# ZeningLin/ViBERTgrid-PyTorch

Hardware: AMD Instinct MI355X
Metric: training docs/sec, 512x512 img + seq_len 512, bert-base+resnet34; 1/2/4/8 GPU (higher is better)
Workload: dtype f32

## Files before the change

### include/vbg.h

```cpp
#ifndef VBG_H
#define VBG_H

#ifdef __cplusplus
extern "C" {
#endif

#define VBG_VERSION 100

int vbg_version(void);

enum {
    VBG_OP_DENSE_K = 0,
    VBG_OP_DENSE_R = 1,
    VBG_OP_CONV_K = 2,
    VBG_OP_CONV_R = 3,
    VBG_OP_WT_R = 4
};
enum { VBG_EPI_NONE = 0, VBG_EPI_RELU = 1, VBG_EPI_GELU_DUAL = 2 ,
       VBG_EPI_MUL_GELU_GRAD = 3  };

typedef struct vbg_conv_geo {
    int Hs, Ws, Cs;
    int Hr, Wr;
    int kh, kw, stride, pad;
// ... 40 lines not shown
    const unsigned short* A; long long a_plane; long long lda;
    const unsigned short* B; long long b_plane; long long ldb;
    float* C; long long ldc; float* C2; const float* bias;
    unsigned short* Cp; long long c_plane; long long ldp;
    int epi; float alpha; int accumulate;
    int splitk;
    int tile;
    int trans;
    int ngroups;
    vbg_plane_group grp[VBG_PLANE_MAX_GROUPS];
    float* colsum;
    int form;
    unsigned short* Cq; long long q_plane; long long ldq;
    const unsigned* a_amax;
    unsigned* c_amax;
    const unsigned* cq_ref_in; const unsigned* cq_l1_in; float cq_mul; unsigned* cq_ref_out;
} vbg_plane_gemm_desc;
typedef struct vbg_l1_entry { const float* w; long long ld; int rows, cols; } vbg_l1_entry;
int vbg_col_l1_max(const vbg_l1_entry* table_dev, int n, int max_cols, unsigned* out, void* stream);
int vbg_plane_gemm(const vbg_plane_gemm_desc* desc, void* stream);
int vbg_plane_gemm_timed(const vbg_plane_gemm_desc* desc, void* stream, void* start_event, void* stop_event);
int vbg_split_planes(const float* x, long long ldx, int rows, int cols, unsigned short* out, int ldp, long long plane, int relu,
                     float* colsum_accum, void* stream);
int vbg_split_planes_t(const float* x, long long ldx, int rows, int cols, unsigned short* out, int ldp, long long plane,
                       void* stream);
int vbg_split_planes_pair(const float* x, long long ldx, int rows, int cols, unsigned short* out, int ldp, long long plane,
                          const unsigned* amax, float* colsum_accum, void* stream);
int vbg_split_planes_t_batched(const float* src, unsigned short* dst, const long long* tbl_dev, int njobs, int total_tiles,
                               long long plane, void* stream);
int vbg_split_planes_pair_t_batched(const float* src, unsigned short* dst, const long long* tbl_dev, int njobs, int total_tiles,
                                    long long plane, void* stream);

enum { VBG_ATTN_FWD = 0, VBG_ATTN_DQ = 1, VBG_ATTN_DKV = 2 };
typedef struct vbg_attn_desc {
    int mode, heads, ntasks, max_len;
    const int* tasks; const int* seq_len; const int* seq_row0; const int* pad_off; long long ntok_pad;
    const unsigned short* qkv; long long qkv_plane, qkv_ld;
    const unsigned short* dO; long long do_plane, do_ld;
    float* out; long long ldo;
    float* lse; float* delta;
    unsigned short* out_planes; long long op_plane, op_ld;
    float* kbar; long long ldk;
    const float* o;
    const unsigned* mask_q; const unsigned* mask_k; const long long* mask_off;
    float scale, keep_scale;
    unsigned* out_amax;
    unsigned short* out_pair; long long oq_plane, oq_ld;
    int form;
    const unsigned* do_amax;
} vbg_attn_desc;
int vbg_attn(const vbg_attn_desc* desc, void* stream);
unsigned vbg_attn_drop_thr16(float drop_p);
int vbg_attn_mask(const int* seq_len, const long long* mask_off, int nseq, int heads, int maxlen, float drop_p,
                  unsigned long long seed, unsigned long long stream_id, unsigned* mask_q, unsigned* mask_k, void* stream);
int vbg_attn_mask_layers(const int* seq_len, const long long* mask_off, int nseq, int heads, int maxlen, float drop_p,
                         unsigned long long seed, unsigned long long stream_id0, unsigned long long stream_id_stride, int nlayers,
                         long long layer_words, unsigned* mask_q, unsigned* mask_k, void* stream);

int vbg_colsum(const float* x, long long ld, int M, int N, float* out, int accumulate, void* stream);
int vbg_colsum_f64(const float* x, long long ld, int M, int N, float* out, int accumulate, double* ws, void* stream);

int vbg_conv3x3_split(int B, int H, int W, int Cs, int N);
int vbg_conv3x3(const float* x, const float* w, const float* bias, float* y, double* stats, int stats_slots, int B, int H, int W,
                int Cs, int N, int accumulate, int form, const unsigned* x_amax, float* split_slab, unsigned* split_tickets,
                int nsplit, void* stream);
#define VBG_AMAX_WORDS 64
#define VBG_AMAX_STRIDE 32
int vbg_amax(const float* x, long long n, unsigned* amax, void* stream);
int vbg_conv3x3_wflip(const float* w, int Cout, int Cin, float* out, void* stream);

typedef struct vbg_conv3_wprep_entry {
    const float* w;
    void* out;
    int Cout, Cin, flip, bn;
} vbg_conv3_wprep_entry;
long long vbg_conv3x3_wprep_bytes(int Cout, int Cin, int flip, int bn);
int vbg_conv3x3_wprep(const vbg_conv3_wprep_entry* table_dev, const vbg_conv3_wprep_entry* table_host, int n, void* stream);
int vbg_conv3x3_pw(const float* x, const void* w_planes, const float* bias, float* y, double* stats, int stats_slots, int B, int H, int W,
                   int Cs, int N, int accumulate, const unsigned* x_amax, float* split_slab, unsigned* split_tickets, int nsplit,
                   int bn, void* stream);
int vbg_conv3x3_pw_amp(const float* x, const void* w_planes, const float* bias, float* y, double* stats, int stats_slots, int B, int H, int W,
                       int Cs, int N, int accumulate, const unsigned* x_amax, float* split_slab, unsigned* split_tickets, int nsplit,
                       int bn, void* stream);

int vbg_conv3x3_wgrad_strips(int B, int H, int W, int Cs, int Cout);
int vbg_conv3x3_wgrad(const float* dy, const float* x, float* dw, float* slab, int B, int H, int W, int Cs, int Cout, int form,
                      const unsigned* dy_amax, const unsigned* x_amax, void* stream);

int vbg_im2col(const float* x, int B, int H, int W, int C, int kh, int kw, int stride, int pad, int Kpad,
               float* out, void* stream);

int vbg_normalize_resize(const float* img, int h, int w, int oh, int ow, const float* h_mean3, const float* h_std3,
                         float* batch_nhwc, int b, int H, int W, void* stream);
int vbg_rescale_boxes(const long long* in, int S, float ratio_h, float ratio_w, int* out, void* stream);

int vbg_embed_ln_fwd(const int* ids, const int* pos_ids, int ntok, int hidden, const float* word, const float* pos,
                     const float* type0, const float* gamma, const float* beta, float eps, float drop_p,
                     unsigned long long seed, unsigned long long stream_id, float* out, float* xhat, float* rstd,
                     void* stream);
int vbg_embed_ln_bwd(const float* dout, const float* xhat, const float* rstd, const int* ids, const int* pos_ids,
                     int ntok, int hidden, const float* gamma, float drop_p, unsigned long long seed,
                     unsigned long long stream_id, float* dword, float* dpos, float* dtype0, float* dgamma,
                     float* dbeta, void* stream);
int vbg_dropout_add_ln_fwd(const float* x, const float* res, int rows, int hidden, const float* gamma,
                           const float* beta, float eps, float drop_p, unsigned long long seed,
                           unsigned long long stream_id, float* y, float* xhat, float* rstd, void* stream);
int vbg_dropout_add_ln_fwd_planes(const float* x, const float* res, int rows, int hidden, const float* gamma,
                                  const float* beta, float eps, float drop_p, unsigned long long seed,
                                  unsigned long long stream_id, float* y, float* xhat, float* rstd, unsigned short* y_planes, int ldp,
                                  long long plane, unsigned short* y_pair, int ldq, long long qplane, void* stream);
int vbg_ln_bwd_ws_rows(int rows);
int vbg_dropout_add_ln_bwd(const float* dy, const float* xhat, const float* rstd, int rows, int hidden,
                           const float* gamma, float drop_p, unsigned long long seed, unsigned long long stream_id,
                           float* dx, float* dres, float* dgamma, float* dbeta, float* slots_ws, unsigned* dx_amax, void* stream);
int vbg_dropout_add_ln_bwd_planes(const float* dy, const float* xhat, const float* rstd, int rows, int hidden,
                                  const float* gamma, float drop_p, unsigned long long seed, unsigned long long stream_id,
                                  unsigned short* dx_planes, int ldp, long long plane, float* dres, float* dgamma, float* dbeta,
                                  float* dbias_accum, float* slots3_ws, void* stream);
int vbg_dropout_add_ln_bwd_pair(const float* dy, const float* xhat, const float* rstd, int rows, int hidden,
                                const float* gamma, float drop_p, unsigned long long seed, unsigned long long stream_id,
                                unsigned short* dx_pair, int ldp, long long plane, float* dres, float* dgamma, float* dbeta,
                                float* dbias_accum, float* slots3_ws, const unsigned* dy_amax, unsigned* dx_amax, unsigned* dx_bound,
                                void* stream);
int vbg_softmax_fwd(float* s, const long long* off, const int* len, const int* ldp, int ngroups, int heads,
                    int maxlen, float scale, float drop_p, unsigned long long seed, unsigned long long stream_id,
                    void* stream);
int vbg_softmax_bwd(const float* p, float* dp, const long long* off, const int* len, const int* ldp, int ngroups,
                    int heads, int maxlen, float scale, float drop_p, void* stream);
int vbg_row_softmax(const float* x, int rows, int cols, float* y, void* stream);
int vbg_gelu_bwd(const float* h, float* dg_inout, long long n, void* stream);
int vbg_relu_bwd(const float* y, float* dy_inout, long long n, void* stream);

typedef struct vbg_planes_ref { unsigned short* buf; long long plane, ld; } vbg_planes_ref;
typedef struct vbg_bert_layer_fwd_desc {
    int ntok, hidden, inter, heads;
    float eps, drop_p; unsigned long long seed, stream_id0;
    int form_qkv, form_attn, form_ao, form_ffn;
    int tile_qkv, tile_ao, tile_ffn1, tile_ffn2;
    int ntasks, max_len; const int* tasks; const int* seq_len; const int* seq_row0; const int* pad_off; long long ntok_pad;
    const unsigned* mask_q; const unsigned* mask_k; const long long* mask_off; float attn_scale, keep_scale;
    const float* x; vbg_planes_ref xa;
    vbg_planes_ref wqkv, wo, wi, wo2;
    const float* bqkv; const float* bo; const float* bi; const float* bo2; const float* g1; const float* b1; const float* g2; const float* b2;
    vbg_planes_ref pqkv;
    float* ctx; float* lse; float* kbar; vbg_planes_ref pctx, pctxq;
    float* ao; float* x1; float* xhat1; float* rstd1; vbg_planes_ref px1, px1q;
    float* h; vbg_planes_ref pg, pgq;
    float* fo; float* y; float* xhat2; float* rstd2; vbg_planes_ref py, pyq;
} vbg_bert_layer_fwd_desc;
int vbg_bert_layer_fwd(const vbg_bert_layer_fwd_desc* desc, void* stream);

int vbg_seg_reduce_fwd(const float* tok, const int* tok_row, const int* run_start, const int* run_len, int nseg,
                       int hidden, int mode, float* out, void* stream);
int vbg_seg_reduce_bwd(const float* dout, const int* tok_row, const int* run_start, const int* run_len, int nseg,
                       int hidden, int mode, float* dtok_accum, void* stream);

int vbg_owner_map(const int* boxes, const int* box_off, int B, int gh, int gw, int stride, int* owner, void* stream);
int vbg_grid_scatter_fwd(const float* emb, const int* owner, int B, int gh, int gw, int C, int layout, float* grid,
                         void* stream);
int vbg_grid_scatter_bwd(const float* dgrid, const int* owner, const int* boxes, const int* box_doc, int nbox, int gh,
                         int gw, int stride, int C, float* demb_accum, void* stream);
int vbg_label_raster(const int* owner, const int* seg_class, long long ncell, int* pos_neg, int* cls, void* stream);

int vbg_bn_slots(void);
int vbg_bn_stats(const float* x, long long M, int C, double* slots_accum, void* stream);
int vbg_bn_finalize(double* stats, int nslots, int clear_slots, double count, const double* count_dev, int C, float eps, float momentum,
                    float* mean, float* invstd, float* running_mean, float* running_var, void* stream);
int vbg_bn_apply(const float* x, const float* res, long long M, int C, const float* mean, const float* invstd,
                 const float* gamma, const float* beta, int relu, float* y, unsigned* y_amax, void* stream);
int vbg_bn_bwd_reduce(const float* dy, const float* y, const float* x, long long M, int C, const float* mean,
                      const float* invstd, int relu, double* slots_accum, void* stream);
int vbg_bn_bwd_apply(const float* dy, const float* y, const float* x, long long M, int C, const float* mean,
                     const float* invstd, const float* gamma, const double* sums, double count, const double* count_dev,
                     int relu, float* dx,
                     float* dres, float* dgamma_accum, float* dbeta_accum, unsigned* dx_amax, void* stream);
int vbg_bn_apply_fold(const float* x, const float* res, long long M, int C, double* slots, int nslots, double count,
                      const double* count_dev, float eps, float momentum, float* mean, float* invstd, float* running_mean,
                      float* running_var, const float* gamma, const float* beta, int relu, float* y, unsigned* y_amax, void* stream);
int vbg_bn_fold_count(double* slots, int nslots, int clear_slots, int C, double* folded, double count, void* stream);
int vbg_bn_bwd_apply_fold(const float* dy, const float* y, const float* x, long long M, int C, const float* mean,
                          const float* invstd, const float* gamma, double* slots, int nslots, double count, int relu, float* dx,
                          float* dres, float* dgamma_accum, float* dbeta_accum, unsigned* dx_amax, void* stream);
int vbg_bn_param_grad(double* slots, int nslots, int clear_slots, int C, double* folded, float* dgamma_accum, float* dbeta_accum,
                      void* stream);
int vbg_maxpool3x3s2_fwd(const float* x, int B, int H, int W, int C, float* y, int* argmax, void* stream);
int vbg_maxpool3x3s2_bwd(const float* dy, const int* argmax, int B, int Ho, int Wo, int C, int H, int W,
                         float* dx, void* stream);
int vbg_avgpool2_fwd(const float* x, int B, int H, int W, int C, float* y, void* stream);
int vbg_avgpool2_bwd(const float* dy, int B, int H, int W, int C, float* dx, void* stream);
int vbg_upsample2_add(const float* lo, const float* skip, int B, int H, int W, int C, float* y, void* stream);
int vbg_sumpool(const float* hi, int B, int H, int W, int C, int f, float* lo, int accumulate, void* stream);
int vbg_nchw_to_nhwc(const float* x, int B, int C, int HW, float* y, void* stream);
int vbg_nhwc_to_nchw(const float* x, int B, int C, int HW, float* y, void* stream);
int vbg_upsample_nhwc_to_nchw(const float* x, int B, int h, int w, int C, int f, float* y, void* stream);
int vbg_add_inplace(float* a, const float* b, long long n, void* stream);

int vbg_roi_align_fwd(const float* feat, int B, int H, int W, int C, const int* boxes, const int* box_doc, int nroi,
                      int out, float scale, float* y , void* stream);
int vbg_roi_align_bwd(const float* dy, int B, int H, int W, int C, const int* boxes, const int* box_doc, int nroi,
                      int out, float scale, float* dfeat_accum, void* stream);

int vbg_ce_fwd(const float* logits, long long ld, int ncls, const int* elem, const int* labels, long long n,
               const float* weight, int up_shift, int H, int W, float* loss, void* stream);
int vbg_ce_bwd(const float* logits, long long ld, int ncls, const int* elem, const int* labels, long long n,
               const float* weight, const float* gscale_dev, float gmul, int up_shift, int H, int W,
               float* dlogits_accum, void* stream);
long long vbg_compact_ws_bytes(long long n);
int vbg_compact(const int* labels, long long n, int value, int eq, int* out_idx, int* out_count_dev, void* ws,
                long long ws_bytes, void* stream);
long long vbg_sort_ws_bytes(long long n);
int vbg_sort_desc(const float* keys, long long n, float* keys_out, int* idx_out, void* ws, long long ws_bytes,
                  void* stream);
int vbg_gather_f32(const float* src, const int* idx, long long n, float* out, void* stream);
int vbg_gather_i32(const int* src, const int* idx, long long n, int* out, void* stream);
int vbg_sum_f32(const float* x, long long n, float* out_accum, void* stream);

int vbg_gather_rows(const float* src, const int* idx, long long n, int C, float* dst, void* stream);
int vbg_scatter_rows_add(const float* src, const int* idx, long long n, int C, float* dst_accum, void* stream);
int vbg_crf_nll_fwd(const float* emissions, const int* tags, const int* doc_off, int ndoc, const float* trans, int ntag,
                    int start_tag, int stop_tag, float* alpha, float* logz, float* nll, void* stream);
int vbg_crf_nll_bwd(const float* emissions, const int* tags, const int* doc_off, int ndoc, const float* trans, int ntag,
                    int start_tag, int stop_tag, const float* alpha, const float* logz, const float* gout, float* demissions,
                    float* dtrans_accum, void* stream);
int vbg_crf_viterbi(const float* emissions, const int* doc_off, int ndoc, const float* trans, int ntag, int start_tag,
                    int stop_tag, int* backptr, int* path, float* score, void* stream);

int vbg_sgd_step(float* p, const float* g, float* mom, long long n, float lr, float momentum, float wd,
                 int first_step, float grad_scale, void* stream);
int vbg_adamw_step(float* p, const float* g, float* m, float* v, long long n, float lr, float b1, float b2,
                   float eps, float wd, int step, float grad_scale, void* stream);
int vbg_sumsq(const float* g, long long n, float* out_accum, void* stream);
int vbg_scale_inplace(float* x, long long n, float s, void* stream);

#ifdef __cplusplus
}
#endif
#endif
```

### vibertgrid-pytorch_amd/csrc/conv3.hip

```cpp
#include "vbg_common.h"
#include <type_traits>
#include <stdlib.h>
#include "../../include/vbg.h"

namespace vbg {

typedef unsigned c3_u32x4 __attribute__((ext_vector_type(4)));
typedef __bf16 c3_bf16x8 __attribute__((ext_vector_type(8)));
constexpr unsigned C3_INVALID = 0x80000000u;

struct conv3_args {
    const float* X;
    const float* Wt;
    const unsigned short* Wp;
    const float* bias;
    float* Y;
    double* stats;
    int stats_slots;
    int H, W, wsh, Cs, N, M;
    int roi;
    int ksplit, csplit;
    float* slab;
    unsigned* tickets;
    int accumulate;
    const unsigned* a_amax;
};

__device__ __forceinline__ __amdgpu_buffer_rsrc_t c3_rsrc(const float* base) {
    return __builtin_amdgcn_make_buffer_rsrc(const_cast<float*>(base), 0, (int)0x80000000u, 0x00020000);
}
__device__ __forceinline__ float4 c3_load(__amdgpu_buffer_rsrc_t r, unsigned vo) {
    const c3_u32x4 v = __builtin_amdgcn_raw_buffer_load_b128(r, (int)vo, 0, 0);
    return make_float4(__uint_as_float(v[0]), __uint_as_float(v[1]), __uint_as_float(v[2]), __uint_as_float(v[3]));
}
__device__ __forceinline__ void c3_split3(float a, float b, unsigned& hi, unsigned& mid, unsigned& lo) {
    const float ra = a - __uint_as_float(__float_as_uint(a) & 0xffff0000u), rb = b - __uint_as_float(__float_as_uint(b) & 0xffff0000u);
    const float sa = ra - __uint_as_float(__float_as_uint(ra) & 0xffff0000u), sb = rb - __uint_as_float(__float_as_uint(rb) & 0xffff0000u);
    hi = __builtin_amdgcn_perm(__float_as_uint(b), __float_as_uint(a), 0x07060302u);
    mid = __builtin_amdgcn_perm(__float_as_uint(rb), __float_as_uint(ra), 0x07060302u);
    lo = __builtin_amdgcn_perm(__float_as_uint(sb), __float_as_uint(sa), 0x07060302u);
}
typedef _Float16 c3_f16x8 __attribute__((ext_vector_type(8)));
typedef __fp16 c3_f16x2 __attribute__((ext_vector_type(2)));
__device__ __forceinline__ void c3_split2(float a, float b, unsigned& hi, unsigned& lo) {
    typedef float f32x2_t __attribute__((ext_vector_type(2)));
    typedef _Float16 f16x2_t __attribute__((ext_vector_type(2)));
    const f32x2_t v = {a, b};
    const f16x2_t h = __builtin_convertvector(v, f16x2_t);
    const f16x2_t l = __builtin_convertvector((v - __builtin_convertvector(h, f32x2_t)) * 2048.f, f16x2_t);
    hi = __builtin_bit_cast(unsigned, h);
    lo = __builtin_bit_cast(unsigned, l);
}
__device__ __forceinline__ unsigned c3_amax_read(const unsigned* slot) {
    unsigned v = slot[(threadIdx.x & (VBG_AMAX_WORDS - 1)) * VBG_AMAX_STRIDE];
#pragma unroll
    for (int o = 32; o > 0; o >>= 1) v = max(v, (unsigned)__shfl_xor((int)v, o, 64));
    return __builtin_amdgcn_readfirstlane(v);
}
__device__ __forceinline__ float2 c3_pow2_scale(unsigned amax_bits) {
    const int e = (int)((amax_bits >> 23) & 0xffu);
    if (e < 27 || e > 240) return make_float2(1.f, 1.f);
    return make_float2(__uint_as_float((unsigned)(267 - e) << 23), __uint_as_float((unsigned)(e - 13) << 23));
}
template <int M, int NM, int NV, int ND>
struct c3_pipe {
    static __device__ __forceinline__ void run() {
        __builtin_amdgcn_sched_group_barrier(0x008, 1, 0);
        constexpr int v = ((M + 1) * NV) / NM - (M * NV) / NM;
        if constexpr (v > 0) __builtin_amdgcn_sched_group_barrier(0x002, v, 0);
        constexpr int w = ((M + 1) * ND) / NM - (M * ND) / NM;
        if constexpr (w > 0) __builtin_amdgcn_sched_group_barrier(0x200, w, 0);
        if constexpr (M + 1 < NM) c3_pipe<M + 1, NM, NV, ND>::run();
    }
};

template <int M, int NM, int NRD, int NV, int ND>
struct c3_pipe2 {
    static __device__ __forceinline__ void run() {
        __builtin_amdgcn_sched_group_barrier(0x008, 1, 0);
        if constexpr (M < NRD) __builtin_amdgcn_sched_group_barrier(0x100, 1, 0);
        constexpr int v = ((M + 1) * NV) / NM - (M * NV) / NM;
        if constexpr (v > 0) __builtin_amdgcn_sched_group_barrier(0x002, v, 0);
        constexpr int w = ((M + 1) * ND) / NM - (M * ND) / NM;
        if constexpr (w > 0) __builtin_amdgcn_sched_group_barrier(0x200, w, 0);
        if constexpr (M + 1 < NM) c3_pipe2<M + 1, NM, NRD, NV, ND>::run();
    }
};

template <int BM, int BN, bool F16, bool PW = false, bool ONEP = false>
__global__ __launch_bounds__(256, 2) void conv3x3_kernel(const conv3_args p) {
    static_assert(!PW || (F16 && BM == 128), "pre-split weights: the fp16-pair form on 128-pixel tiles");
    static_assert(!ONEP || PW, "the one-product form exists for the pre-split kernels");
    constexpr int NT = 256, SKH = 24;
    constexpr int NSB = 4;
    constexpr int BTILE = 64 * BN;
    constexpr int NDB = BN / 64;
    constexpr int NDBE = (ONEP && NDB == 2) ? 1 : NDB;
    constexpr int TNF = BN / 64;
    constexpr int NBI = BN * 4 / NT;
    constexpr int NPL = F16 ? 2 : 3;
    constexpr int NQ = ONEP ? 1 : NPL;
    constexpr int NAI = BM * 4 / NT;
    constexpr int TM = BM / 64;
    constexpr int AROWS = BM + BM / 8;
    constexpr int PA = AROWS * SKH / 2, PB = BN * SKH / 2;
    constexpr int ASZ = NPL * PA, BSZ = NPL * PB;
    constexpr int CTS = BN + 4;
    constexpr int LOOPSZ = PW ? 2 * ASZ + NSB * BTILE / 4 : 2 * (ASZ + BSZ);
// ... 263 lines not shown
            unsigned* dst = As + buf * ASZ;
#pragma unroll
            for (int i = 0; i < NAI; ++i) {
                const int o = a_lrow[i] * (SKH / 2) + kc / 2;
                *reinterpret_cast<uint2*>(&dst[o]) = sh[i];
                if constexpr (!ONEP) *reinterpret_cast<uint2*>(&dst[o + PA]) = sl[i];
            }
            if (wide && tid < 8) {
                const int o = h_row * (SKH / 2) + kc / 2;
                *reinterpret_cast<uint2*>(&dst[o]) = sh[NAI];
                if constexpr (!ONEP) *reinterpret_cast<uint2*>(&dst[o + PA]) = sl[NAI];
            }
        };
        using p0 = std::integral_constant<int, 0>;
        using p1 = std::integral_constant<int, 1>;
        int bst = 0;
        auto tile = [&](auto par_tag, auto kw_tag, int s) {
            constexpr int P = decltype(par_tag)::value, KW = decltype(kw_tag)::value;
            const int nst = bst + 1 == NSB ? 0 : bst + 1;
            __builtin_amdgcn_sched_barrier(0);
            if constexpr (P == 0) read_frags(p1{}, KW < 2 ? (s & 1) : ((s + 1) & 1), nst, KW < 2 ? KW + 1 : 0);
            else read_frags(p0{}, KW < 2 ? (s & 1) : ((s + 1) & 1), nst, KW < 2 ? KW + 1 : 0);
            if constexpr (P == 0) mma_set(p0{}); else mma_set(p1{});
            if constexpr (KW == 1) split_a();
            constexpr int NM = (ONEP ? 1 : 3) * TM * TNF, NRD = NQ * (TM + TNF);
            c3_pipe2<0, NM, NRD, KW == 1 ? (NAI + 1) * (ONEP ? 6 : 10) : 0, 0>::run();
            __builtin_amdgcn_sched_barrier(0);
            if constexpr (KW == 1) write_a((s + 1) & 1);
            if constexpr (KW == 0) load_a();
            issue_b();
            if constexpr (KW == 0) {
                if (wide) asm volatile("s_waitcnt vmcnt(%0) lgkmcnt(0)" ::"n"((NSB - 2) * NDBE + NAI + 1) : "memory");
                else asm volatile("s_waitcnt vmcnt(%0) lgkmcnt(0)" ::"n"((NSB - 2) * NDBE + NAI) : "memory");
            } else {
                asm volatile("s_waitcnt vmcnt(%0) lgkmcnt(0)" ::"n"((NSB - 2) * NDBE) : "memory");
            }
            __builtin_amdgcn_s_barrier();
            bst = nst;
        };
        read_frags(p0{}, 0, 0, 0);
        asm volatile("s_waitcnt lgkmcnt(0)" ::: "memory");
        __builtin_amdgcn_s_barrier();
        using k0 = std::integral_constant<int, 0>;
        using k1 = std::integral_constant<int, 1>;
        using k2 = std::integral_constant<int, 2>;
        for (int s = 0; s < nsup; s += 2) {
            tile(p0{}, k0{}, s); tile(p1{}, k1{}, s); tile(p0{}, k2{}, s);
            if (s + 1 < nsup) { tile(p1{}, k0{}, s + 1); tile(p0{}, k1{}, s + 1); tile(p1{}, k2{}, s + 1); }
        }
        asm volatile("s_waitcnt vmcnt(0)" ::: "memory");
    } else {
    load_a();
    load_b();
    __syncthreads();
    store_a(0);
    store_b(0);
    __syncthreads();
    int t = 0;
    for (int s = 0; s + 1 < nsup; ++s) {
        k_tile(no_t{}, yes_t{}, s & 1, t & 1, 0); ++t;
        k_tile(no_t{}, yes_t{}, s & 1, t & 1, 1); ++t;
        k_tile(yes_t{}, yes_t{}, s & 1, t & 1, 2); ++t;
    }
    {
        const int s = nsup - 1;
        k_tile(no_t{}, yes_t{}, s & 1, t & 1, 0); ++t;
        k_tile(no_t{}, yes_t{}, s & 1, t & 1, 1); ++t;
        k_tile(no_t{}, no_t{}, s & 1, t & 1, 2);
    }
    }

    const float* bias = p.bias;
    const int accumulate = p.accumulate;
    __syncthreads();
    float* const Ct = reinterpret_cast<float*>(smem);
#pragma unroll
    for (int j = 0; j < TNF; ++j)
#pragma unroll
        for (int i = 0; i < TM; ++i)
#pragma unroll
            for (int r = 0; r < 16; ++r)
                Ct[(wm * (BM / 2) + i * 32 + (r & 3) + 8 * (r >> 2) + 4 * lk) * CTS + wn * (BN / 2) + j * 32 + lr] =
                    ONEP ? acc[i][j][r] * a_sc.y : (F16 ? (acc[i][j][r] + acx[i][j][r] * (1.f / 2048.f)) * a_sc.y : acc[i][j][r]);
    __syncthreads();
    constexpr int QN = BN / 4;
    const float* part = nullptr;
    if (nz > 1) {
        unsigned& ticket_s = smem[SMEM];
        const size_t tile = (size_t)tile_n * gx + tile_m;
        float* const mine = p.slab + (tile * nz + zz) * (size_t)(BM * BN);
        const __amdgpu_buffer_rsrc_t rs = __builtin_amdgcn_make_buffer_rsrc(mine, 0, BM * BN * 4, 0x00020000);
#pragma unroll 4
        for (int q = 0; q < BM * QN / NT; ++q) {
            const int idx = tid + q * NT;
            const int row = idx / QN, c = (idx % QN) * 4;
            const c3_u32x4 v = *reinterpret_cast<const c3_u32x4*>(&Ct[row * CTS + c]);
            __builtin_amdgcn_raw_buffer_store_b128(v, rs, (row * BN + c) * 4, 0, 16 );
        }
        asm volatile("s_waitcnt vmcnt(0)" ::: "memory");
        __syncthreads();
        if (tid == 0) ticket_s = __hip_atomic_fetch_add(p.tickets + tile, 1u, __ATOMIC_RELAXED, __HIP_MEMORY_SCOPE_AGENT);
        __syncthreads();
        if (ticket_s != (unsigned)(nz - 1)) return;
        if (tid == 0) {
            __builtin_amdgcn_fence(__ATOMIC_ACQUIRE, "agent");
            __hip_atomic_store(p.tickets + tile, 0u, __ATOMIC_RELAXED, __HIP_MEMORY_SCOPE_AGENT);
        }
        __syncthreads();
        part = p.slab + tile * nz * (size_t)(BM * BN);
    }
    float4 cs = make_float4(0.f, 0.f, 0.f, 0.f), cq = cs;
#pragma unroll 4
    for (int q = 0; q < BM * QN / NT; ++q) {
        const int idx = tid + q * NT;
        const int row = idx / QN, c = (idx % QN) * 4;
        int gm = m0 + row;
        const int gn = n0 + c;
        if (gn >= N) continue;
        if (roi) {
            const int im = nb + (row >> 6), sy = (row >> 3) & 7, sx = row & 7;
            if (im >= roi || sy == 7 || sx == 7) continue;
            gm = im * 49 + sy * 7 + sx;
        }
        float4 v;
        if (part) {
            v = make_float4(0.f, 0.f, 0.f, 0.f);
            for (int b = 0; b < nz; ++b) {
                const float4 o = *reinterpret_cast<const float4*>(part + (size_t)b * (BM * BN) + row * BN + c);
                v.x += o.x; v.y += o.y; v.z += o.z; v.w += o.w;
            }
        } else {
            v = *reinterpret_cast<const float4*>(&Ct[row * CTS + c]);
        }
        if (bias) { v.x += bias[gn]; v.y += bias[gn + 1]; v.z += bias[gn + 2]; v.w += bias[gn + 3]; }
        float* cp = p.Y + (long long)gm * N + gn;
        if (p.stats) {
            cs.x += v.x; cs.y += v.y; cs.z += v.z; cs.w += v.w;
            cq.x += v.x * v.x; cq.y += v.y * v.y; cq.z += v.z * v.z; cq.w += v.w * v.w;
        }
        if (accumulate) {
            const float4 o = *reinterpret_cast<const float4*>(cp);
            v.x += o.x; v.y += o.y; v.z += o.z; v.w += o.w;
        }
        *reinterpret_cast<float4*>(cp) = v;
    }
    if (p.stats) {
        constexpr int RG = NT / QN;
        float* red = reinterpret_cast<float*>(smem);
        __syncthreads();
        const int rg = tid / QN, c = (tid % QN) * 4;
        *reinterpret_cast<float4*>(&red[(0 * RG + rg) * BN + c]) = cs;
        *reinterpret_cast<float4*>(&red[(1 * RG + rg) * BN + c]) = cq;
        __syncthreads();
        for (int e = tid; e < 2 * BN; e += NT) {
            const int st = e / BN, col = e - st * BN;
            if (n0 + col >= N) continue;
            double acc64 = 0.0;
            for (int g2 = 0; g2 < RG; ++g2) acc64 += (double)red[(st * RG + g2) * BN + col];
            unsafeAtomicAdd(p.stats + (size_t)(tile_m % (unsigned)p.stats_slots) * 2 * N + (size_t)st * N + n0 + col, acc64);
        }
    }
}

__global__ void conv3_wflip_kernel(const float* __restrict__ w, int Cout, int Cin, float* __restrict__ out) {
    __shared__ float t[32][33];
    const int tap = blockIdx.z, co0 = blockIdx.y * 32, ci0 = blockIdx.x * 32;
    const int tx = threadIdx.x, ty = threadIdx.y;
#pragma unroll
    for (int j = 0; j < 4; ++j) {
        const int co = co0 + ty + 8 * j, ci = ci0 + tx;
        t[ty + 8 * j][tx] = (co < Cout && ci < Cin) ? w[((long long)co * 9 + tap) * Cin + ci] : 0.f;
    }
    __syncthreads();
#pragma unroll
    for (int j = 0; j < 4; ++j) {
        const int ci = ci0 + ty + 8 * j, co = co0 + tx;
        if (ci < Cin && co < Cout) out[((long long)ci * 9 + (8 - tap)) * Cout + co] = t[tx][ty + 8 * j];
    }
}

__global__ __launch_bounds__(256) void conv3_wprep_kernel(const vbg_conv3_wprep_entry* __restrict__ tab) {
    const vbg_conv3_wprep_entry e = tab[blockIdx.y];
    const int bn = e.bn, rows = e.flip ? e.Cin : e.Cout, K = e.flip ? e.Cout : e.Cin;
    const int gpb = bn * 2;
    const long long g = (long long)blockIdx.x * 256 + threadIdx.x;
    const long long nblocks = (long long)((rows + bn - 1) / bn) * 9 * (K / 16);
    if (g >= nblocks * gpb) return;
    const long long blk = g / gpb;
    const int in = (int)(g - blk * gpb);
    const int row32 = in & 31, half = (in >> 5) & 1, rb = in >> 6;
    const int chunk = (int)(blk % (K / 16));
    const int tap = (int)((blk / (K / 16)) % 9);
    const int tile = (int)(blk / ((long long)(K / 16) * 9));
    const int r = tile * bn + rb * 32 + row32;
    const int k0 = chunk * 16 + half * 8;
    float v[8];
    if (r < rows) {
        if (!e.flip) {
            const float4* src = reinterpret_cast<const float4*>(e.w + ((long long)r * 9 + tap) * e.Cin + k0);
            const float4 a = src[0], b = src[1];
            v[0] = a.x; v[1] = a.y; v[2] = a.z; v[3] = a.w; v[4] = b.x; v[5] = b.y; v[6] = b.z; v[7] = b.w;
        } else {
#pragma unroll
            for (int j = 0; j < 8; ++j) v[j] = e.w[((long long)(k0 + j) * 9 + (8 - tap)) * e.Cin + r];
        }
    } else {
#pragma unroll
        for (int j = 0; j < 8; ++j) v[j] = 0.f;
    }
    uint4 h, l;
    c3_split2(v[0], v[1], h.x, l.x);
    c3_split2(v[2], v[3], h.y, l.y);
    c3_split2(v[4], v[5], h.z, l.z);
    c3_split2(v[6], v[7], h.w, l.w);
    unsigned char* dst = reinterpret_cast<unsigned char*>(e.out) + blk * (64ll * bn) + (long long)rb * 1024 + half * 512 + row32 * 16;
    *reinterpret_cast<uint4*>(dst) = h;
    *reinterpret_cast<uint4*>(dst + 32 * bn) = l;
}

// ... 269 lines not shown
    VBG_CHECK_ARG(dy && x && dw && B > 0 && H > 0 && (roi || (W >= 16 && W % 16 == 0)));
    VBG_CHECK_ARG(form == 0 || ((form == 1 || form == 2) && dy_amax && x_amax));
    VBG_CHECK_ARG(Cs % 32 == 0 && Cout % 64 == 0);
    VBG_CHECK_ARG((((uintptr_t)x) & 15) == 0 && (((uintptr_t)dy) & 15) == 0);
    VBG_CHECK_ARG((long long)(3 * W + 18) * Cs < (1ll << 28) && (long long)16 * Cout < (1ll << 28));
    const long long M = (long long)B * H * W;
    VBG_CHECK_ARG(M < (1ll << 31));
    vbg::conv3w_args a;
    a.dY = dy; a.X = x; a.dW = dw; a.slab = slab; a.H = H; a.W = W; a.Cs = Cs; a.Cout = Cout;
    a.dy_amax = dy_amax; a.x_amax = x_amax;
    a.roi = roi ? 1 : 0;
    a.nchunks = roi ? B * 4 : (int)(M / 16);
    const bool wide = Cout % 128 == 0;
    VBG_CHECK_ARG(wide || Cs % 64 == 0);
    const int nsplit = vbg_conv3x3_wgrad_strips(B, H, W, Cs, Cout);
    VBG_CHECK_ARG(nsplit >= 1 && (!slab || (((uintptr_t)slab) & 15) == 0) && (((uintptr_t)dw) & 15) == 0);
    a.per = (a.nchunks + nsplit - 1) / nsplit;
    if (roi) {
        VBG_CHECK_ARG(wide);
        if (form == 2) { VBG_LAUNCH((vbg::conv3x3_wgrad_kernel<4, true, true, true>), dim3(nsplit, Cs / 32, Cout / 128), dim3(256), 0, (hipStream_t)stream, a); }
        else if (form == 1) { VBG_LAUNCH((vbg::conv3x3_wgrad_kernel<4, true, true>), dim3(nsplit, Cs / 32, Cout / 128), dim3(256), 0, (hipStream_t)stream, a); }
        else { VBG_LAUNCH((vbg::conv3x3_wgrad_kernel<4, false, true>), dim3(nsplit, Cs / 32, Cout / 128), dim3(256), 0, (hipStream_t)stream, a); }
    } else if (wide) {
        if (form == 2) { VBG_LAUNCH((vbg::conv3x3_wgrad_kernel<4, true, false, true>), dim3(nsplit, Cs / 32, Cout / 128), dim3(256), 0, (hipStream_t)stream, a); }
        else if (form == 1) { VBG_LAUNCH((vbg::conv3x3_wgrad_kernel<4, true>), dim3(nsplit, Cs / 32, Cout / 128), dim3(256), 0, (hipStream_t)stream, a); }
        else { VBG_LAUNCH((vbg::conv3x3_wgrad_kernel<4, false>), dim3(nsplit, Cs / 32, Cout / 128), dim3(256), 0, (hipStream_t)stream, a); }
    } else {
        if (form == 2) { VBG_LAUNCH((vbg::conv3x3_wgrad_kernel<2, true, false, true>), dim3(nsplit, Cs / 64, Cout / 64), dim3(256), 0, (hipStream_t)stream, a); }
        else if (form == 1) { VBG_LAUNCH((vbg::conv3x3_wgrad_kernel<2, true>), dim3(nsplit, Cs / 64, Cout / 64), dim3(256), 0, (hipStream_t)stream, a); }
        else { VBG_LAUNCH((vbg::conv3x3_wgrad_kernel<2, false>), dim3(nsplit, Cs / 64, Cout / 64), dim3(256), 0, (hipStream_t)stream, a); }
    }
    if (slab) {
        const long long n4 = (long long)Cout * 9 * Cs / 4;
        static const int par_from = getenv("VBG_CONV3W_REDUCE_PAR") ? atoi(getenv("VBG_CONV3W_REDUCE_PAR")) : 32;
        if (par_from > 0 && nsplit >= par_from)
            hipLaunchKernelGGL(vbg::conv3_wgrad_reduce_par_kernel, dim3((unsigned)((n4 + 63) / 64)), dim3(1024), 0, (hipStream_t)stream,
                               reinterpret_cast<const float4*>(slab), nsplit, n4, reinterpret_cast<float4*>(dw));
        else
            hipLaunchKernelGGL(vbg::conv3_wgrad_reduce_kernel, dim3((unsigned)((n4 + 255) / 256)), dim3(256), 0, (hipStream_t)stream,
                               reinterpret_cast<const float4*>(slab), nsplit, n4, reinterpret_cast<float4*>(dw));
    }
    VBG_LAUNCH_RET();
}

extern "C" int vbg_conv3x3_split(int B, int H, int W, int Cs, int N) {
    static const int forced = getenv("VBG_CONV3_SPLIT_Z") ? atoi(getenv("VBG_CONV3_SPLIT_Z")) : 0;
    if (W < 16 || (W & (W - 1)) != 0 || ((long long)H * W) % 128 != 0 || N % 128 != 0 || Cs % 16 != 0 || W >= 128) return 1;
    const long long tiles = ((long long)B * H * W / 128) * (N / 128);
    if (tiles >= 240 || tiles < 4) return 1;
    int nz = tiles * 3 >= 256 ? 3 : tiles * 4 >= 256 ? 4 : tiles * 6 >= 256 ? 6 : 12;
    if (tiles < 16) nz = 4;
    if (forced > 0) nz = forced;
    const int cs = nz % 3 == 0 ? nz / 3 : nz;
    if (Cs % cs != 0 || (Cs / cs) % 16 != 0) return 1;
    return nz;
}

static int conv3_pw_bn(int rows) { return (rows % 128 != 0 && rows % 64 == 0) ? 64 : 128; }

extern "C" long long vbg_conv3x3_wprep_bytes(int Cout, int Cin, int flip, int bn_req) {
    const int rows = flip ? Cin : Cout, K = flip ? Cout : Cin;
    if (rows <= 0 || K <= 0 || K % 16 != 0 || !(bn_req == 0 || bn_req == 64 || bn_req == 128)) return 0;
    const int bn = bn_req ? bn_req : conv3_pw_bn(rows);
    return (long long)((rows + bn - 1) / bn) * 9 * (K / 16) * 64 * bn;
}

extern "C" int vbg_conv3x3_wprep(const vbg_conv3_wprep_entry* table_dev, const vbg_conv3_wprep_entry* table_host, int n, void* stream) {
    VBG_CHECK_ARG(n >= 0 && (n == 0 || (table_dev && table_host)));
    if (n == 0) return VBG_OK;
    long long most = 0;
    for (int i = 0; i < n; ++i) {
        const vbg_conv3_wprep_entry& e = table_host[i];
        const int rows = e.flip ? e.Cin : e.Cout, K = e.flip ? e.Cout : e.Cin;
        VBG_CHECK_ARG(e.w && e.out && rows > 0 && K > 0 && K % 16 == 0 && e.Cin % 8 == 0 && (e.bn == 64 || e.bn == 128));
        VBG_CHECK_ARG((((uintptr_t)e.w) & 15) == 0 && (((uintptr_t)e.out) & 15) == 0);
        const long long groups = (long long)((rows + e.bn - 1) / e.bn) * 9 * (K / 16) * e.bn * 2;
        most = groups > most ? groups : most;
    }
    VBG_CHECK_ARG((most + 255) / 256 < (1ll << 31));
    VBG_LAUNCH(vbg::conv3_wprep_kernel, dim3((unsigned)((most + 255) / 256), (unsigned)n), dim3(256), 0, (hipStream_t)stream, table_dev);
    VBG_LAUNCH_RET();
}

static int conv3x3_impl(const float* x, const float* w, const unsigned short* wp, const float* bias, float* y, double* stats, int stats_slots,
                        int B, int H, int W, int Cs, int N, int accumulate, int form, const unsigned* x_amax, float* split_slab,
                        unsigned* split_tickets, int nsplit, void* stream, int bn_req = 0);

extern "C" int vbg_conv3x3(const float* x, const float* w, const float* bias, float* y, double* stats, int stats_slots, int B, int H,
                           int W, int Cs, int N, int accumulate, int form, const unsigned* x_amax, float* split_slab,
                           unsigned* split_tickets, int nsplit, void* stream) {
    VBG_CHECK_ARG(w);
    return conv3x3_impl(x, w, nullptr, bias, y, stats, stats_slots, B, H, W, Cs, N, accumulate, form, x_amax, split_slab, split_tickets, nsplit, stream);
}

extern "C" int vbg_conv3x3_pw(const float* x, const void* w_planes, const float* bias, float* y, double* stats, int stats_slots, int B, int H,
                              int W, int Cs, int N, int accumulate, const unsigned* x_amax, float* split_slab, unsigned* split_tickets,
                              int nsplit, int bn, void* stream) {
    VBG_CHECK_ARG(w_planes && (((uintptr_t)w_planes) & 15) == 0 && (bn == 0 || bn == 64 || bn == 128));
    return conv3x3_impl(x, nullptr, (const unsigned short*)w_planes, bias, y, stats, stats_slots, B, H, W, Cs, N, accumulate, 1, x_amax, split_slab,
                        split_tickets, nsplit, stream, bn);
}

extern "C" int vbg_conv3x3_pw_amp(const float* x, const void* w_planes, const float* bias, float* y, double* stats, int stats_slots, int B, int H,
                                  int W, int Cs, int N, int accumulate, const unsigned* x_amax, float* split_slab, unsigned* split_tickets,
                                  int nsplit, int bn, void* stream) {
    VBG_CHECK_ARG(w_planes && (((uintptr_t)w_planes) & 15) == 0 && (bn == 0 || bn == 64 || bn == 128));
    return conv3x3_impl(x, nullptr, (const unsigned short*)w_planes, bias, y, stats, stats_slots, B, H, W, Cs, N, accumulate, 2, x_amax, split_slab,
                        split_tickets, nsplit, stream, bn);
}

static int conv3x3_impl(const float* x, const float* w, const unsigned short* wp, const float* bias, float* y, double* stats, int stats_slots,
                        int B, int H, int W, int Cs, int N, int accumulate, int form, const unsigned* x_amax, float* split_slab,
                        unsigned* split_tickets, int nsplit, void* stream, int bn_req) {
    VBG_CHECK_ARG(form == 0 || form == 1 || (form == 2 && wp));
    VBG_CHECK_ARG(bn_req == 0 || wp);
    VBG_CHECK_ARG(!x_amax || form >= 1);
    VBG_CHECK_ARG(x && (w || wp) && y && B > 0 && H > 0);
    const bool roi = H == 7 && W == 7;
    VBG_CHECK_ARG(roi || (W >= 16 && W <= 4096 && (W & (W - 1)) == 0));
    VBG_CHECK_ARG(roi || ((long long)H * W) % 64 == 0);
    VBG_CHECK_ARG((long long)H * W * Cs < (1ll << 29) && (!roi || (long long)B * 49 * Cs < (1ll << 29)));
    VBG_CHECK_ARG(Cs >= 16 && Cs % 16 == 0 && N >= 4 && N % 4 == 0);
    VBG_CHECK_ARG((((uintptr_t)x) & 15) == 0 && (((uintptr_t)w) & 15) == 0 && (((uintptr_t)y) & 15) == 0);
    VBG_CHECK_ARG(!stats || (stats_slots >= 1 && !accumulate));
    vbg::conv3_args a;
    a.X = x; a.Wt = w; a.Wp = wp; a.bias = bias; a.Y = y; a.stats = stats; a.stats_slots = stats_slots;
    a.H = H; a.W = W; a.wsh = roi ? 3 : 31 - __builtin_clz((unsigned)W); a.Cs = Cs; a.N = N;
    const long long M = (long long)B * H * W;
    VBG_CHECK_ARG(M < (1ll << 31));
    a.M = (int)M; a.accumulate = accumulate; a.a_amax = x_amax; a.roi = roi ? B : 0;
    const bool split = nsplit > 1;
    VBG_CHECK_ARG(nsplit >= 1 && (!split || (split_slab && split_tickets && !roi && N % (bn_req ? bn_req : 128) == 0 && ((long long)H * W) % 128 == 0)));
    a.ksplit = split && nsplit % 3 == 0 ? 3 : 1;
    a.csplit = split ? nsplit / a.ksplit : 1;
    a.slab = split_slab; a.tickets = split_tickets;
    VBG_CHECK_ARG(Cs % a.csplit == 0 && (Cs / a.csplit) % 16 == 0 && (((uintptr_t)split_slab) & 15) == 0);
    auto is_big = [&](int bn_) { return roi || (((long long)H * W) % 128 == 0 && ((M / 128) * vbg::cdiv(N, bn_) >= 240 || W >= 128)); };
    const bool n64 = bn_req ? bn_req == 64 : (N % 128 != 0 && N % 64 == 0 && is_big(64));
    const int bn = n64 ? 64 : 128;
    const bool big = bn_req ? (roi || ((long long)H * W) % 128 == 0) : (split || is_big(bn));
    const dim3 g(roi ? (unsigned)((B + 1) / 2) : (unsigned)(M / (big ? 128 : 64)), (unsigned)vbg::cdiv(N, bn), (unsigned)nsplit);
    if (wp) {
        VBG_CHECK_ARG(big && (bn_req || bn == conv3_pw_bn(N)));
        if (form == 2) {
            if (n64) { VBG_LAUNCH((vbg::conv3x3_kernel<128, 64, true, true, true>), g, dim3(256), 0, (hipStream_t)stream, a); }
            else { VBG_LAUNCH((vbg::conv3x3_kernel<128, 128, true, true, true>), g, dim3(256), 0, (hipStream_t)stream, a); }
        } else {
            if (n64) { VBG_LAUNCH((vbg::conv3x3_kernel<128, 64, true, true>), g, dim3(256), 0, (hipStream_t)stream, a); }
            else { VBG_LAUNCH((vbg::conv3x3_kernel<128, 128, true, true>), g, dim3(256), 0, (hipStream_t)stream, a); }
        }
        VBG_LAUNCH_RET();
    }
    if (n64) {
        if (form == 1) { VBG_LAUNCH((vbg::conv3x3_kernel<128, 64, true>), g, dim3(256), 0, (hipStream_t)stream, a); }
        else { VBG_LAUNCH((vbg::conv3x3_kernel<128, 64, false>), g, dim3(256), 0, (hipStream_t)stream, a); }
    } else if (form == 1) {
        if (big) { VBG_LAUNCH((vbg::conv3x3_kernel<128, 128, true>), g, dim3(256), 0, (hipStream_t)stream, a); }
        else { VBG_LAUNCH((vbg::conv3x3_kernel<64, 128, true>), g, dim3(256), 0, (hipStream_t)stream, a); }
    } else {
        if (big) { VBG_LAUNCH((vbg::conv3x3_kernel<128, 128, false>), g, dim3(256), 0, (hipStream_t)stream, a); }
        else { VBG_LAUNCH((vbg::conv3x3_kernel<64, 128, false>), g, dim3(256), 0, (hipStream_t)stream, a); }
    }
    VBG_LAUNCH_RET();
}

extern "C" int vbg_conv3x3_wflip(const float* w, int Cout, int Cin, float* out, void* stream) {
    VBG_CHECK_ARG(w && out && Cout > 0 && Cin > 0);
    dim3 g((unsigned)vbg::cdiv(Cin, 32), (unsigned)vbg::cdiv(Cout, 32), 9);
    VBG_LAUNCH(vbg::conv3_wflip_kernel, g, dim3(32, 8), 0, (hipStream_t)stream, w, Cout, Cin, out);
    VBG_LAUNCH_RET();
}
```

### vibertgrid-pytorch_amd/csrc/convaux.hip

```cpp
#include "vbg_common.h"
#include "../../include/vbg.h"

namespace vbg {

static inline int ew_grid(long long n, int block) {
    long long g = (n + block - 1) / block;
    if (g > 256 * 8) g = 256 * 8;
    if (g < 1) g = 1;
    return (int)g;
}

constexpr int BN_SLOTS = 32;
template <bool BWD>
__global__ __launch_bounds__(256) void bn_reduce_kernel(const float* __restrict__ a, const float* __restrict__ y,
                                                        const float* __restrict__ x, long long M, int C,
                                                        const float* __restrict__ mean, const float* __restrict__ invstd,
                                                        int relu, int rows_per_block, double* out) {
    __shared__ double sh[2][256][4];
    const int C4 = C >> 2;
    const int QB = min(C4, 64);
    const int RL = 256 / QB;
    const int q = threadIdx.x % QB, rl = threadIdx.x / QB;
    const int cq = blockIdx.x * 64 + q;
    const long long r0 = (long long)blockIdx.y * rows_per_block;
// ... 128 lines not shown
                                    float* __restrict__ dres, unsigned* amax) {
    if (count_dev) count = count_dev[0];
    float mx = 0.f;
    const float icnt = (float)(1.0 / count);
    const long long total = M * C4;
    const long long stride = (long long)gridDim.x * blockDim.x;
    for (long long i = (long long)blockIdx.x * blockDim.x + threadIdx.x; i < total; i += stride) {
        const int c4 = (int)(i % C4), c = c4 * 4;
        float4 g = reinterpret_cast<const float4*>(dy)[i];
        if (relu) {
            const float4 yv = reinterpret_cast<const float4*>(y)[i];
            g.x = yv.x > 0.f ? g.x : 0.f; g.y = yv.y > 0.f ? g.y : 0.f; g.z = yv.z > 0.f ? g.z : 0.f; g.w = yv.w > 0.f ? g.w : 0.f;
        }
        const float4 xv = reinterpret_cast<const float4*>(x)[i];
        const float4 mu = reinterpret_cast<const float4*>(mean)[c4], is = reinterpret_cast<const float4*>(invstd)[c4];
        const float4 ga = reinterpret_cast<const float4*>(gamma)[c4];
        float4 o;
        o.x = ga.x * is.x * (g.x - (float)sums[c + 0] * icnt - (xv.x - mu.x) * is.x * ((float)sums[C + c + 0] * icnt));
        o.y = ga.y * is.y * (g.y - (float)sums[c + 1] * icnt - (xv.y - mu.y) * is.y * ((float)sums[C + c + 1] * icnt));
        o.z = ga.z * is.z * (g.z - (float)sums[c + 2] * icnt - (xv.z - mu.z) * is.z * ((float)sums[C + c + 2] * icnt));
        o.w = ga.w * is.w * (g.w - (float)sums[c + 3] * icnt - (xv.w - mu.w) * is.w * ((float)sums[C + c + 3] * icnt));
        reinterpret_cast<float4*>(dx)[i] = o;
        if (dres) reinterpret_cast<float4*>(dres)[i] = g;
        mx = fmaxf(fmaxf(mx, fmaxf(fabsf(o.x), fabsf(o.y))), fmaxf(fabsf(o.z), fabsf(o.w)));
    }
    if (amax) amax_publish(mx, amax);
}

__device__ __forceinline__ void amax_publish_at(float mx, unsigned* amax, unsigned block_id) {
    __shared__ float amax_sh2[16];
#pragma unroll
    for (int o = 32; o > 0; o >>= 1) mx = fmaxf(mx, __shfl_xor(mx, o, 64));
    if ((threadIdx.x & 63) == 0) amax_sh2[threadIdx.x >> 6] = mx;
    __syncthreads();
    if (threadIdx.x == 0) {
        for (int w = 1; w < (int)(blockDim.x >> 6); ++w) mx = fmaxf(mx, amax_sh2[w]);
        const unsigned bits = __float_as_uint(mx);
        unsigned* word = amax + (block_id & (VBG_AMAX_WORDS - 1)) * VBG_AMAX_STRIDE;
        if (bits > __hip_atomic_load(word, __ATOMIC_RELAXED, __HIP_MEMORY_SCOPE_AGENT)) atomicMax(word, bits);
    }
}

__global__ __launch_bounds__(256) void bn_apply_fold_kernel(const float* __restrict__ x, const float* __restrict__ res, long long M, int C,
                                                            double* __restrict__ slots, int nslots, double count,
                                                            const double* __restrict__ count_dev, float eps, float momentum,
                                                            float* __restrict__ mean_out, float* __restrict__ invstd_out,
                                                            float* __restrict__ running_mean, float* __restrict__ running_var,
                                                            const float* __restrict__ gamma, const float* __restrict__ beta, int relu,
                                                            int rows_per_block, float* __restrict__ y, unsigned* amax) {
    __shared__ double fold[128];
    __shared__ __attribute__((aligned(16))) float cst[4][64];
    const int tid = threadIdx.x, c0 = blockIdx.y * 64;
    if (count_dev) count = count_dev[0];
    if (tid < 128) fold[tid] = fold_slots(slots, nslots, C, (tid >> 6) * C + c0 + (tid & 63), false);
    __syncthreads();
    if (tid < 64) {
        const int c = c0 + tid;
        const double m = fold[tid] / count;
        double var = fold[64 + tid] / count - m * m;
        if (var < 0.0) var = 0.0;
        const float mf = (float)m, isf = (float)(1.0 / sqrt(var + (double)eps));
        cst[0][tid] = mf; cst[1][tid] = isf; cst[2][tid] = gamma[c]; cst[3][tid] = beta[c];
        if (blockIdx.x == 0) {
            mean_out[c] = mf;
            invstd_out[c] = isf;
            if (running_mean) {
                const double unbiased = count > 1.0 ? var * count / (count - 1.0) : var;
                running_mean[c] = (1.f - momentum) * running_mean[c] + momentum * mf;
                running_var[c] = (1.f - momentum) * running_var[c] + momentum * (float)unbiased;
            }
        }
    }
    __syncthreads();
    const int q = tid & 15, rl = tid >> 4, C4 = C >> 2, cq = blockIdx.y * 16 + q;
    const float4 mu = reinterpret_cast<const float4*>(cst[0])[q], is = reinterpret_cast<const float4*>(cst[1])[q];
    const float4 ga = reinterpret_cast<const float4*>(cst[2])[q], be = reinterpret_cast<const float4*>(cst[3])[q];
    const long long r0 = (long long)blockIdx.x * rows_per_block, r1 = min(M, r0 + rows_per_block);
    float mx = 0.f;
#pragma unroll 4
    for (long long r = r0 + rl; r < r1; r += 16) {
        const long long i = r * C4 + cq;
        const float4 xv = reinterpret_cast<const float4*>(x)[i];
        float4 o;
        o.x = (xv.x - mu.x) * is.x * ga.x + be.x; o.y = (xv.y - mu.y) * is.y * ga.y + be.y;
        o.z = (xv.z - mu.z) * is.z * ga.z + be.z; o.w = (xv.w - mu.w) * is.w * ga.w + be.w;
        if (res) {
            const float4 rv = reinterpret_cast<const float4*>(res)[i];
            o.x += rv.x; o.y += rv.y; o.z += rv.z; o.w += rv.w;
        }
        if (relu) { o.x = fmaxf(o.x, 0.f); o.y = fmaxf(o.y, 0.f); o.z = fmaxf(o.z, 0.f); o.w = fmaxf(o.w, 0.f); }
        reinterpret_cast<float4*>(y)[i] = o;
        mx = fmaxf(fmaxf(mx, fmaxf(fabsf(o.x), fabsf(o.y))), fmaxf(fabsf(o.z), fabsf(o.w)));
    }
    if (amax) amax_publish_at(mx, amax, blockIdx.x + blockIdx.y * gridDim.x);
}

__global__ __launch_bounds__(256) void bn_bwd_apply_fold_kernel(const float* __restrict__ dy, const float* __restrict__ y,
                                                                const float* __restrict__ x, long long M, int C,
                                                                const float* __restrict__ mean, const float* __restrict__ invstd,
                                                                const float* __restrict__ gamma, double* __restrict__ slots, int nslots,
                                                                double count, int relu, int rows_per_block, float* __restrict__ dx,
                                                                float* __restrict__ dres, float* dgamma, float* dbeta, unsigned* amax) {
    __shared__ double fold[128];
    __shared__ __attribute__((aligned(16))) float cst[5][64];
    const int tid = threadIdx.x, c0 = blockIdx.y * 64;
    if (tid < 128) fold[tid] = fold_slots(slots, nslots, C, (tid >> 6) * C + c0 + (tid & 63), false);
    __syncthreads();
    const float icnt = (float)(1.0 / count);
    if (tid < 64) {
        const int c = c0 + tid;
        const double sg = fold[tid], sgx = fold[64 + tid];
        cst[0][tid] = mean[c]; cst[1][tid] = invstd[c]; cst[2][tid] = gamma[c];
        cst[3][tid] = (float)sg * icnt; cst[4][tid] = (float)sgx * icnt;
        if (blockIdx.x == 0) {
            if (dbeta) dbeta[c] += (float)sg;
            if (dgamma) dgamma[c] += (float)sgx;
        }
    }
    __syncthreads();
    const int q = tid & 15, rl = tid >> 4, C4 = C >> 2, cq = blockIdx.y * 16 + q;
    const float4 mu = reinterpret_cast<const float4*>(cst[0])[q], is = reinterpret_cast<const float4*>(cst[1])[q];
    const float4 ga = reinterpret_cast<const float4*>(cst[2])[q], s0 = reinterpret_cast<const float4*>(cst[3])[q];
    const float4 s1 = reinterpret_cast<const float4*>(cst[4])[q];
    const long long r0 = (long long)blockIdx.x * rows_per_block, r1 = min(M, r0 + rows_per_block);
    float mx = 0.f;
#pragma unroll 4
    for (long long r = r0 + rl; r < r1; r += 16) {
        const long long i = r * C4 + cq;
        float4 g = reinterpret_cast<const float4*>(dy)[i];
        if (relu) {
            const float4 yv = reinterpret_cast<const float4*>(y)[i];
            g.x = yv.x > 0.f ? g.x : 0.f; g.y = yv.y > 0.f ? g.y : 0.f; g.z = yv.z > 0.f ? g.z : 0.f; g.w = yv.w > 0.f ? g.w : 0.f;
        }
        const float4 xv = reinterpret_cast<const float4*>(x)[i];
        float4 o;
        o.x = ga.x * is.x * (g.x - s0.x - (xv.x - mu.x) * is.x * s1.x);
        o.y = ga.y * is.y * (g.y - s0.y - (xv.y - mu.y) * is.y * s1.y);
        o.z = ga.z * is.z * (g.z - s0.z - (xv.z - mu.z) * is.z * s1.z);
        o.w = ga.w * is.w * (g.w - s0.w - (xv.w - mu.w) * is.w * s1.w);
        reinterpret_cast<float4*>(dx)[i] = o;
        if (dres) reinterpret_cast<float4*>(dres)[i] = g;
        mx = fmaxf(fmaxf(mx, fmaxf(fabsf(o.x), fabsf(o.y))), fmaxf(fabsf(o.z), fabsf(o.w)));
    }
    if (amax) amax_publish_at(mx, amax, blockIdx.x + blockIdx.y * gridDim.x);
}

__global__ __launch_bounds__(256) void amax_kernel(const float* __restrict__ x, long long n, unsigned* amax) {
    const long long n4 = n / 4, stride = (long long)gridDim.x * blockDim.x;
    float mx = 0.f;
    for (long long i = (long long)blockIdx.x * blockDim.x + threadIdx.x; i < n4; i += stride) {
        const float4 v = reinterpret_cast<const float4*>(x)[i];
        mx = fmaxf(fmaxf(mx, fmaxf(fabsf(v.x), fabsf(v.y))), fmaxf(fabsf(v.z), fabsf(v.w)));
    }
    if (blockIdx.x == 0 && threadIdx.x < (int)(n - n4 * 4)) mx = fmaxf(mx, fabsf(x[n4 * 4 + threadIdx.x]));
    amax_publish(mx, amax);
}

__global__ void bn_param_grad_kernel(double* __restrict__ slots, int nslots, int clear, int C, double* __restrict__ folded, float* dgamma,
                                     float* dbeta, double tail = -1.0) {
    const int c = blockIdx.x * blockDim.x + threadIdx.x;
    if (c == 0 && folded && tail >= 0.0) folded[2 * C] = tail;
    if (c >= C) return;
    const double sg = fold_slots(slots, nslots, C, c, clear), sgx = fold_slots(slots, nslots, C, C + c, clear);
    if (folded) { folded[c] = sg; folded[C + c] = sgx; }
    if (dbeta) dbeta[c] += (float)sg;
    if (dgamma) dgamma[c] += (float)sgx;
}

__global__ void maxpool_fwd_kernel(const float* __restrict__ x, int B, int H, int W, int C, int Ho, int Wo,
                                   float* __restrict__ y, int* __restrict__ argmax) {
    const long long total = (long long)B * Ho * Wo * C;
    const long long stride = (long long)gridDim.x * blockDim.x;
    for (long long i = (long long)blockIdx.x * blockDim.x + threadIdx.x; i < total; i += stride) {
        const int c = (int)(i % C);
        long long t = i / C;
        const int ox = (int)(t % Wo); t /= Wo;
        const int oy = (int)(t % Ho);
        const int b = (int)(t / Ho);
        float best = -INFINITY;
        int bi = -1;
        for (int dy = 0; dy < 3; ++dy) {
            const int iy = oy * 2 - 1 + dy;
            if (iy < 0 || iy >= H) continue;
            for (int dx = 0; dx < 3; ++dx) {
                const int ix = ox * 2 - 1 + dx;
                if (ix < 0 || ix >= W) continue;
                const float v = x[(((long long)b * H + iy) * W + ix) * C + c];
                if (v > best || bi < 0) { best = v; bi = iy * W + ix; }
            }
        }
        y[i] = best;
        argmax[i] = bi;
    }
}

__global__ void maxpool_bwd_kernel(const float* __restrict__ dy, const int* __restrict__ argmax, int B, int Ho, int Wo, int C4, int H,
                                   int W, float* __restrict__ dx) {
    const long long total = (long long)B * H * W * C4;
    const long long stride = (long long)gridDim.x * blockDim.x;
    for (long long i = (long long)blockIdx.x * blockDim.x + threadIdx.x; i < total; i += stride) {
        const int c4 = (int)(i % C4);
        long long t = i / C4;
        const int x = (int)(t % W); t /= W;
        const int y = (int)(t % H);
        const int b = (int)(t / H);
        const int me = y * W + x;
        float4 g = make_float4(0.f, 0.f, 0.f, 0.f);
        for (int oy = y >> 1; oy <= ((y + 1) >> 1); ++oy) {
            if (oy >= Ho) continue;
            for (int ox = x >> 1; ox <= ((x + 1) >> 1); ++ox) {
                if (ox >= Wo) continue;
                const long long o = (((long long)b * Ho + oy) * Wo + ox) * C4 + c4;
                const int4 am = reinterpret_cast<const int4*>(argmax)[o];
                const float4 d = reinterpret_cast<const float4*>(dy)[o];
                g.x += am.x == me ? d.x : 0.f; g.y += am.y == me ? d.y : 0.f;
                g.z += am.z == me ? d.z : 0.f; g.w += am.w == me ? d.w : 0.f;
            }
// ... 180 lines not shown

extern "C" int vbg_bn_stats(const float* x, long long M, int C, double* stats_accum, void* stream) {
    VBG_CHECK_ARG(x && stats_accum && M >= 0 && C > 0 && C % 4 == 0 && ALIGNED16(x));
    VBG_CHECK_ARG(C / 4 <= 64 ? (256 % (C / 4) == 0) : (C / 4) % 64 == 0);
    if (M == 0) return VBG_OK;
    const int rpb = bn_rows_per_block(M, C);
    VBG_LAUNCH((bn_reduce_kernel<false>), dim3(cdiv(C / 4, 64), cdiv(M, rpb)), dim3(256), 0, S_, x, nullptr, nullptr, M, C, nullptr,
               nullptr, 0, rpb, stats_accum);
    VBG_LAUNCH_RET();
}

extern "C" int vbg_bn_slots(void) { return BN_SLOTS; }

extern "C" int vbg_bn_finalize(double* stats, int nslots, int clear_slots, double count, const double* count_dev, int C, float eps, float momentum,
                               float* mean, float* invstd, float* running_mean, float* running_var, void* stream) {
    VBG_CHECK_ARG(stats && nslots >= 1 && mean && invstd && C > 0 && (count > 0 || count_dev) &&
                  ((running_mean == nullptr) == (running_var == nullptr)));
    VBG_LAUNCH(bn_finalize_kernel, dim3(cdiv(C, 256)), dim3(256), 0, S_, stats, nslots, clear_slots, count, count_dev, C, eps, momentum, mean,
                       invstd, running_mean, running_var);
    VBG_LAUNCH_RET();
}

extern "C" int vbg_bn_apply(const float* x, const float* res, long long M, int C, const float* mean, const float* invstd,
                            const float* gamma, const float* beta, int relu, float* y, unsigned* y_amax, void* stream) {
    VBG_CHECK_ARG(x && mean && invstd && gamma && beta && y && M >= 0 && C > 0 && C % 4 == 0);
    VBG_CHECK_ARG(ALIGNED16(x) && ALIGNED16(y) && ALIGNED16(mean) && ALIGNED16(invstd) && ALIGNED16(gamma) && ALIGNED16(beta) &&
                  (!res || ALIGNED16(res)));
    if (M == 0) return VBG_OK;
    VBG_LAUNCH(bn_apply_kernel, dim3(ew_grid(M * (C / 4), 256)), dim3(256), 0, S_, x, res, M, C / 4, mean, invstd, gamma,
                       beta, relu, y, y_amax);
    VBG_LAUNCH_RET();
}

extern "C" int vbg_bn_bwd_reduce(const float* dy, const float* y, const float* x, long long M, int C, const float* mean,
                                 const float* invstd, int relu, double* sums_accum, void* stream) {
    VBG_CHECK_ARG(dy && x && mean && invstd && sums_accum && M >= 0 && C > 0 && (!relu || y) && C % 4 == 0);
    VBG_CHECK_ARG(ALIGNED16(dy) && ALIGNED16(x) && ALIGNED16(mean) && ALIGNED16(invstd) && (!relu || ALIGNED16(y)));
    VBG_CHECK_ARG(C / 4 <= 64 ? (256 % (C / 4) == 0) : (C / 4) % 64 == 0);
    if (M == 0) return VBG_OK;
    const int rpb = bn_rows_per_block(M, C);
    VBG_LAUNCH((bn_reduce_kernel<true>), dim3(cdiv(C / 4, 64), cdiv(M, rpb)), dim3(256), 0, S_, dy, y, x, M, C, mean, invstd, relu,
               rpb, sums_accum);
    VBG_LAUNCH_RET();
}

extern "C" int vbg_bn_bwd_apply(const float* dy, const float* y, const float* x, long long M, int C, const float* mean,
                                const float* invstd, const float* gamma, const double* sums, double count,
                                const double* count_dev, int relu, float* dx, float* dres, float* dgamma_accum,
                                float* dbeta_accum, unsigned* dx_amax, void* stream) {
    VBG_CHECK_ARG(dy && x && mean && invstd && gamma && sums && dx && M >= 0 && C > 0 && (count > 0 || count_dev) && (!relu || y));
    VBG_CHECK_ARG(C % 4 == 0 && ALIGNED16(dy) && ALIGNED16(x) && ALIGNED16(dx) && ALIGNED16(mean) && ALIGNED16(invstd) &&
                  ALIGNED16(gamma) && (!relu || ALIGNED16(y)) && (!dres || ALIGNED16(dres)));
    if (M > 0) VBG_LAUNCH(bn_bwd_apply_kernel, dim3(ew_grid(M * (C / 4), 256)), dim3(256), 0, S_, dy, y, x, M, C / 4, C, mean, invstd,
                          gamma, sums, count, count_dev, relu, dx, dres, dx_amax);
    if (dgamma_accum && dbeta_accum)
        VBG_LAUNCH(bn_param_grad_kernel, dim3(cdiv(C, 256)), dim3(256), 0, S_, const_cast<double*>(sums), 1, 0, C, (double*)nullptr, dgamma_accum, dbeta_accum, -1.0);
    VBG_LAUNCH_RET();
}

static inline int bn_fold_rows(long long M, int C) {
    long long r = cdiv(M * (C / 64), 1536);
    if (r < 64) r = 64;
    return (int)(cdiv(r, 16) * 16);
}

extern "C" int vbg_bn_apply_fold(const float* x, const float* res, long long M, int C, double* slots, int nslots, double count,
                                 const double* count_dev, float eps, float momentum, float* mean, float* invstd, float* running_mean,
                                 float* running_var, const float* gamma, const float* beta, int relu, float* y, unsigned* y_amax, void* stream) {
    VBG_CHECK_ARG(x && y && slots && mean && invstd && gamma && beta && M > 0 && C > 0 && C % 64 == 0 && nslots >= 1 && (count > 0 || count_dev));
    VBG_CHECK_ARG((running_mean == nullptr) == (running_var == nullptr) && ALIGNED16(x) && ALIGNED16(y) && (!res || ALIGNED16(res)));
    const int rpb = bn_fold_rows(M, C);
    VBG_LAUNCH(bn_apply_fold_kernel, dim3(cdiv(M, rpb), C / 64), dim3(256), 0, S_, x, res, M, C, slots, nslots, count, count_dev, eps, momentum, mean, invstd,
               running_mean, running_var, gamma, beta, relu, rpb, y, y_amax);
    VBG_LAUNCH_RET();
}

extern "C" int vbg_bn_bwd_apply_fold(const float* dy, const float* y, const float* x, long long M, int C, const float* mean,
                                     const float* invstd, const float* gamma, double* slots, int nslots, double count, int relu, float* dx,
                                     float* dres, float* dgamma_accum, float* dbeta_accum, unsigned* dx_amax, void* stream) {
    VBG_CHECK_ARG(dy && x && mean && invstd && gamma && slots && dx && M > 0 && C > 0 && C % 64 == 0 && nslots >= 1 && count > 0 && (!relu || y));
    VBG_CHECK_ARG(((dgamma_accum == nullptr) == (dbeta_accum == nullptr)) && ALIGNED16(dy) && ALIGNED16(x) && ALIGNED16(dx) &&
                  (!relu || ALIGNED16(y)) && (!dres || ALIGNED16(dres)));
    const int rpb = bn_fold_rows(M, C);
    VBG_LAUNCH(bn_bwd_apply_fold_kernel, dim3(cdiv(M, rpb), C / 64), dim3(256), 0, S_, dy, y, x, M, C, mean, invstd, gamma, slots, nslots, count,
               relu, rpb, dx, dres, dgamma_accum, dbeta_accum, dx_amax);
    VBG_LAUNCH_RET();
}

extern "C" int vbg_amax(const float* x, long long n, unsigned* amax, void* stream) {
    VBG_CHECK_ARG(n >= 0 && amax);
    if (n == 0) return VBG_OK;
    VBG_CHECK_ARG(x && ALIGNED16(x));
    VBG_LAUNCH(amax_kernel, dim3(ew_grid((n + 3) / 4, 256 * 8)), dim3(256), 0, S_, x, n, amax);
    VBG_LAUNCH_RET();
}

extern "C" int vbg_bn_param_grad(double* slots, int nslots, int clear_slots, int C, double* folded, float* dgamma_accum,
                                 float* dbeta_accum, void* stream) {
    VBG_CHECK_ARG(slots && nslots >= 1 && C > 0 && ((dgamma_accum == nullptr) == (dbeta_accum == nullptr)) && (folded || dgamma_accum));
    VBG_LAUNCH(bn_param_grad_kernel, dim3(cdiv(C, 256)), dim3(256), 0, S_, slots, nslots, clear_slots, C, folded, dgamma_accum, dbeta_accum, -1.0);
    VBG_LAUNCH_RET();
}

extern "C" int vbg_bn_fold_count(double* slots, int nslots, int clear_slots, int C, double* folded, double count, void* stream) {
    VBG_CHECK_ARG(slots && folded && nslots >= 1 && C > 0 && count >= 0);
    VBG_LAUNCH(bn_param_grad_kernel, dim3(cdiv(C, 256)), dim3(256), 0, S_, slots, nslots, clear_slots, C, folded, (float*)nullptr, (float*)nullptr, count);
    VBG_LAUNCH_RET();
}

extern "C" int vbg_maxpool3x3s2_fwd(const float* x, int B, int H, int W, int C, float* y, int* argmax, void* stream) {
    VBG_CHECK_ARG(x && y && argmax && B >= 0 && H > 0 && W > 0 && C > 0);
    const int Ho = (H + 2 - 3) / 2 + 1, Wo = (W + 2 - 3) / 2 + 1;
    const long long total = (long long)B * Ho * Wo * C;
    if (total == 0) return VBG_OK;
    VBG_LAUNCH(maxpool_fwd_kernel, dim3(ew_grid(total, 256)), dim3(256), 0, S_, x, B, H, W, C, Ho, Wo, y, argmax);
    VBG_LAUNCH_RET();
}

extern "C" int vbg_maxpool3x3s2_bwd(const float* dy, const int* argmax, int B, int Ho, int Wo, int C, int H, int W,
                                    float* dx_zeroed, void* stream) {
    VBG_CHECK_ARG(dy && argmax && dx_zeroed && B >= 0 && Ho > 0 && Wo > 0 && C > 0 && C % 4 == 0);
    VBG_CHECK_ARG(ALIGNED16(dy) && ALIGNED16(argmax) && ALIGNED16(dx_zeroed) && Ho == (H + 2 - 3) / 2 + 1 && Wo == (W + 2 - 3) / 2 + 1);
    const long long total = (long long)B * Ho * Wo * C;
    if (total == 0) return VBG_OK;
    VBG_LAUNCH(maxpool_bwd_kernel, dim3(ew_grid((long long)B * H * W * (C / 4), 256)), dim3(256), 0, S_, dy, argmax, B, Ho, Wo, C / 4, H, W,
               dx_zeroed);
    VBG_LAUNCH_RET();
}

extern "C" int vbg_upsample2_add(const float* lo, const float* skip, int B, int H, int W, int C, float* y, void* stream) {
    VBG_CHECK_ARG(lo && skip && y && H % 2 == 0 && W % 2 == 0 && C % 4 == 0 && ALIGNED16(lo) && ALIGNED16(skip) && ALIGNED16(y));
    const long long total = (long long)B * H * W * (C / 4);
    if (total == 0) return VBG_OK;
    VBG_LAUNCH(upsample2_add_kernel, dim3(ew_grid(total, 256)), dim3(256), 0, S_, lo, skip, B, H, W, C / 4, y);
    VBG_LAUNCH_RET();
}

extern "C" int vbg_avgpool2_fwd(const float* x, int B, int H, int W, int C, float* y, void* stream) {
    VBG_CHECK_ARG(x && y && B >= 0 && H >= 2 && W >= 2 && C > 0 && C % 4 == 0 && ALIGNED16(x) && ALIGNED16(y));
    const long long total = (long long)B * (H / 2) * (W / 2) * (C / 4);
    if (total == 0) return VBG_OK;
    VBG_LAUNCH((avgpool2_kernel<false>), dim3(ew_grid(total, 256)), dim3(256), 0, S_, x, B, H, W, C / 4, y);
    VBG_LAUNCH_RET();
}

extern "C" int vbg_avgpool2_bwd(const float* dy, int B, int H, int W, int C, float* dx, void* stream) {
    VBG_CHECK_ARG(dy && dx && B >= 0 && H >= 2 && W >= 2 && C > 0 && C % 4 == 0 && ALIGNED16(dy) && ALIGNED16(dx));
    const long long total = (long long)B * H * W * (C / 4);
    if (total == 0) return VBG_OK;
    VBG_LAUNCH((avgpool2_kernel<true>), dim3(ew_grid(total, 256)), dim3(256), 0, S_, dy, B, H, W, C / 4, dx);
    VBG_LAUNCH_RET();
}

extern "C" int vbg_sumpool(const float* hi, int B, int H, int W, int C, int f, float* lo, int accumulate, void* stream) {
    VBG_CHECK_ARG(hi && lo && f >= 1 && H % f == 0 && W % f == 0 && C % 4 == 0 && ALIGNED16(hi) && ALIGNED16(lo));
    const long long total = (long long)B * (H / f) * (W / f) * (C / 4);
    if (total == 0) return VBG_OK;
    VBG_LAUNCH(sumpool_kernel, dim3(ew_grid(total, 256)), dim3(256), 0, S_, hi, B, H, W, C / 4, f, lo, accumulate);
    VBG_LAUNCH_RET();
}

extern "C" int vbg_nchw_to_nhwc(const float* x, int B, int C, int HW, float* y, void* stream) {
    VBG_CHECK_ARG(x && y && B >= 0 && C > 0 && HW > 0);
    if (B == 0) return VBG_OK;
    VBG_LAUNCH(transpose_kernel, dim3(cdiv(HW, 32), cdiv(C, 32), B), dim3(256), 0, S_, x, C, HW, y);
    VBG_LAUNCH_RET();
}

// ... 44 lines not shown
```

### vibertgrid-pytorch_amd/csrc/vbg_common.h

```cpp
#pragma once
#include <hip/hip_runtime.h>
#include <stdint.h>

#define VBG_OK 0
#define VBG_EARG (-1)

#define VBG_CHECK_ARG(cond) do { if (!(cond)) return VBG_EARG; } while (0)
#define VBG_LAUNCH(...) do { (void)hipGetLastError(); hipLaunchKernelGGL(__VA_ARGS__); } while (0)
#define VBG_LAUNCH_RET() do { hipError_t e__ = hipGetLastError(); return e__ == hipSuccess ? VBG_OK : (int)e__; } while (0)

typedef float f32x4 __attribute__((ext_vector_type(4)));
typedef float f32x16 __attribute__((ext_vector_type(16)));

namespace vbg {

static inline int cdiv(long a, long b) { return (int)((a + b - 1) / b); }

__device__ __forceinline__ float wave_sum(float v) {
#pragma unroll
    for (int o = 32; o > 0; o >>= 1) v += __shfl_xor(v, o, 64);
    return v;
}
__device__ __forceinline__ float wave_max(float v) {
#pragma unroll
    for (int o = 32; o > 0; o >>= 1) v = fmaxf(v, __shfl_xor(v, o, 64));
    return v;
}
__device__ __forceinline__ float block_sum(float v, float* sh) {
    const int lane = threadIdx.x & 63, w = threadIdx.x >> 6, nw = (blockDim.x + 63) >> 6;
    v = wave_sum(v);
    __syncthreads();
    if (lane == 0) sh[w] = v;
    __syncthreads();
    float r = 0.f;
    for (int i = 0; i < nw; ++i) r += sh[i];
    return r;
}
__device__ __forceinline__ float block_max(float v, float* sh) {
    const int lane = threadIdx.x & 63, w = threadIdx.x >> 6, nw = (blockDim.x + 63) >> 6;
    v = wave_max(v);
    __syncthreads();
    if (lane == 0) sh[w] = v;
    __syncthreads();
    float r = sh[0];
    for (int i = 1; i < nw; ++i) r = fmaxf(r, sh[i]);
    return r;
}

__host__ __device__ __forceinline__ uint32_t rng_u32(uint64_t seed, uint64_t stream, uint64_t idx) {
    uint64_t z = seed + 0x9E3779B97F4A7C15ull * (stream + 1) + idx * 0xBF58476D1CE4E5B9ull;
    z ^= z >> 30; z *= 0xBF58476D1CE4E5B9ull;
    z ^= z >> 27; z *= 0x94D049BB133111EBull;
    z ^= z >> 31;
    return (uint32_t)(z >> 16);
}
__host__ __device__ __forceinline__ bool rng_keep(uint64_t seed, uint64_t stream, uint64_t idx, uint32_t drop_thresh) {
    return rng_u32(seed, stream, idx) >= drop_thresh;
}
static inline uint32_t drop_threshold(float p) {
    double t = (double)p * 4294967296.0;
    if (t <= 0) return 0u;
    if (t >= 4294967295.0) return 4294967295u;
    return (uint32_t)t;
}

__device__ __forceinline__ float vbg_erff(float a) {
    const float t = fabsf(a), s = a * a;
    float r = fmaf(-1.72853470e-5f, t, 3.83197126e-4f);
    const float u = fmaf(-3.88396438e-3f, t, 2.42546219e-2f);
    r = fmaf(r, s, u);
    r = fmaf(r, t, -1.06777877e-1f);
    r = fmaf(r, t, -6.34846687e-1f);
    r = fmaf(r, t, -1.28717512e-1f);
    r = fmaf(r, t, -t);
    const float big = 1.0f - __expf(r);
    float q = -5.96761703e-4f;
    q = fmaf(q, s, 4.99119423e-3f);
    q = fmaf(q, s, -2.67681349e-2f);
    q = fmaf(q, s, 1.12819925e-1f);
    q = fmaf(q, s, -3.76125336e-1f);
    q = fmaf(q, s, 1.28379166e-1f);
    q = fmaf(q, t, t);
    return copysignf(t > 0.927734375f ? big : q, a);
}
__device__ __forceinline__ float gelu_erf(float x) { return 0.5f * x * (1.0f + vbg_erff(x * 0.70710678118654752440f)); }
__device__ __forceinline__ float gelu_erf_grad(float x) {
    const float cdf = 0.5f * (1.0f + vbg_erff(x * 0.70710678118654752440f));
    const float pdf = 0.39894228040143267794f * __expf(-0.5f * x * x);
    return cdf + x * pdf;
}

}

#if defined(__HIPCC__)
#ifndef VBG_AMAX_WORDS
#define VBG_AMAX_WORDS 64
#define VBG_AMAX_STRIDE 32
#endif
__device__ __forceinline__ unsigned vbg_amax_read(const unsigned* slot) {
    unsigned v = slot[(threadIdx.x & (VBG_AMAX_WORDS - 1)) * VBG_AMAX_STRIDE];
#pragma unroll
    for (int o = 32; o > 0; o >>= 1) v = max(v, (unsigned)__shfl_xor((int)v, o, 64));
    return __builtin_amdgcn_readfirstlane(v);
}
__device__ __forceinline__ float2 vbg_pow2_scale(unsigned amax_bits) {
    const int e = (int)((amax_bits >> 23) & 0xffu);
    if (e < 27 || e > 240) return make_float2(1.f, 1.f);
    return make_float2(__uint_as_float((unsigned)(267 - e) << 23), __uint_as_float((unsigned)(e - 13) << 23));
}
__device__ __forceinline__ void vbg_amax_publish(float mx, unsigned* amax, float* sh16) {
#pragma unroll
    for (int o = 32; o > 0; o >>= 1) mx = fmaxf(mx, __shfl_xor(mx, o, 64));
    if ((threadIdx.x & 63) == 0) sh16[threadIdx.x >> 6] = mx;
    __syncthreads();
    if (threadIdx.x == 0) {
        for (int w = 1; w < (int)(blockDim.x >> 6); ++w) mx = fmaxf(mx, sh16[w]);
        const unsigned bits = __float_as_uint(mx);
        const unsigned lin = blockIdx.x + gridDim.x * (blockIdx.y + gridDim.y * blockIdx.z);
        unsigned* word = amax + (lin & (VBG_AMAX_WORDS - 1)) * VBG_AMAX_STRIDE;
        if (bits > __hip_atomic_load(word, __ATOMIC_RELAXED, __HIP_MEMORY_SCOPE_AGENT)) atomicMax(word, bits);
    }
}
#endif
```

### vibertgrid-pytorch_amd/vbg/functions.py

```python
import torch
import torch.distributed as dist

from . import ops
from .lib import ATTN_DKV, ATTN_DQ, ATTN_FWD, EPI_GELU_DUAL, EPI_MUL_GELU_GRAD, EPI_NONE, EPI_RELU, OP_DENSE_K, OP_DENSE_R

f32 = torch.float32


def ohwi(w):
    v = w.permute(0, 2, 3, 1)
    return v if v.is_contiguous() else v.contiguous()


def oihw_grad_like(dw_ohwi):
    return dw_ohwi.permute(0, 3, 1, 2)


def _c(t):
    return t if t.is_contiguous() else t.contiguous()


GRAD_READY = [None]
SIDE_OK = [False]


def wgrad_dest(w):
    if getattr(w, "_vbg_sunk", False):
        g = w.grad
        if g is None:
            g = w._vbg_flat[0].attach(w)
        return g
    return None


def sinks(w) -> bool:
    return getattr(w, "_vbg_sunk", False)


def wgrad_done(w):
    if GRAD_READY[0] is not None:
        GRAD_READY[0](w)


def _bias_grad(b_param, dy2d):
    dst = wgrad_dest(b_param)
    if dst is not None:
        ops.colsum(dy2d, out=dst, accumulate=True)
        wgrad_done(b_param)
        return None
    return ops.colsum(dy2d)


def _affine_dest(gamma_param, beta_param):
    dg, db = wgrad_dest(gamma_param), wgrad_dest(beta_param)
    if dg is not None and db is not None:
        return dg, db, True
    return torch.zeros_like(gamma_param), torch.zeros_like(beta_param), False


def _affine_done(gamma_param, beta_param, dg, db, sunk):
    if sunk:
        wgrad_done(gamma_param)
        wgrad_done(beta_param)
        return None, None
    return dg, db


def _amax_tag(x):
    tag = getattr(x, "_vbg_amax", None)
    if tag is None:
        return None
    slot, version = tag
    return slot if x._version == version else None


class SyncCtx:
    group = None
    before = None
    seq = 0
    last = None
    force = False
    direct = None

    @classmethod
    def active(cls):
        return dist.is_available() and dist.is_initialized() and (dist.get_world_size(cls.group) > 1 or cls.force)

    @classmethod
    def all_reduce(cls, t):
        if cls.before is not None:
            cls.before()
        cls.seq += 1
        cls.last = (cls.seq, t.numel())
        if cls.direct is not None and t.is_cuda:
            cls.direct.all_reduce_(t)
        else:
            dist.all_reduce(t, group=cls.group)


def _linear_wgrad(w_param, dy, x):
    dst = wgrad_dest(w_param)
    if dst is not None:
        ops.linear_wgrad(dy, x, dst, accumulate=True)
        wgrad_done(w_param)
        return None
    dw = torch.empty_like(w_param)
    ops.linear_wgrad(dy, x, dw, accumulate=False)
    return dw


def _split_with_bias_grad(b_param, dy2d):
    dst = wgrad_dest(b_param)
    if dst is not None:
        pl = ops.split_planes(dy2d, colsum_out=dst)
        wgrad_done(b_param)
        return pl, None
    return ops.split_planes(dy2d), ops.colsum(dy2d)


def _plane_wgrad(w_param, dy, x):
    N, K = dy.shape[1], x.shape[1]
    pa, pb = ops.split_planes_t(dy), ops.split_planes_t(x)
    dst = wgrad_dest(w_param)
    if dst is not None:
        ops.plane_gemm(pa, pb, dst, accumulate=True, tile=ops._wgrad_tile(N, K))
        wgrad_done(w_param)
        return None
    dw = torch.empty_like(w_param)
    ops.plane_gemm(pa, pb, dw, tile=ops._wgrad_tile(N, K))
    return dw


class LinearFn(torch.autograd.Function):

    @staticmethod
    def forward(ctx, x, w, b, relu):
        x = _c(x)
        y = ops.linear_fwd(x, w, b, EPI_RELU if relu else EPI_NONE)
        ctx.relu = relu
        ctx.has_bias = b is not None
        ctx.w_ref, ctx.b_ref = w, b
        ctx.save_for_backward(x, w, y if relu else None)
        return y

    @staticmethod
    def backward(ctx, dy):
        x, w, y = ctx.saved_tensors
        dy = _c(dy)
        if ctx.relu:
            dy = ops.relu_bwd_(y, dy.clone())
        dx = ops.linear_dgrad(dy, w) if ctx.needs_input_grad[0] else None
        dw = _linear_wgrad(ctx.w_ref, dy, x)
        db = _bias_grad(ctx.b_ref, dy) if ctx.has_bias else None
        return dx, dw, db, None


# ... 78 lines not shown


def _conv_wgrad_any(dy, x, col, w4_shape, stride, pad, w_param=None, dy_amax=None, x_amax=None):
    dst = wgrad_dest(w_param) if w_param is not None else None
    if dst is not None:
        dw = ohwi(dst)
        assert dw.data_ptr() == dst.data_ptr()
        if col is not None:
            Cout, kh, kw, Cin = w4_shape
            K = kh * kw * Cin
            sk = ops._pick_splitk(Cout, K, col.shape[0])
            ops.gemm_raw(Cout, K, col.shape[0], dy, Cout, OP_DENSE_R, col, col.shape[1], OP_DENSE_R, dw, K, accumulate=True, splitk=sk)
        else:
            ops.conv2d_wgrad(dy, x, dw, stride, pad, accumulate=True, dy_amax=dy_amax, x_amax=x_amax)
        wgrad_done(w_param)
        return None
    dw = torch.empty(w4_shape, device=dy.device, dtype=f32)
    if col is not None:
        Cout, kh, kw, Cin = w4_shape
        K = kh * kw * Cin
        Mpix = col.shape[0]
        sk = ops._pick_splitk(Cout, K, Mpix)
        if sk > 1:
            dw.zero_()
        ops.gemm_raw(Cout, K, Mpix, dy, Cout, OP_DENSE_R, col, col.shape[1], OP_DENSE_R, dw, K, accumulate=sk > 1, splitk=sk)
    else:
        ops.conv2d_wgrad(dy, x, dw, stride, pad, accumulate=False, dy_amax=dy_amax, x_amax=x_amax)
    return oihw_grad_like(dw)


class ConvFn(torch.autograd.Function):

    @staticmethod
    def forward(ctx, x, w, b, stride, pad):
        ctx.x_amax = _amax_tag(x)
        x = _c(x)
        w4 = ohwi(w)
        y, col, _ = _conv_any(x, w4, stride, pad, b, w_owner=w, x_amax=ctx.x_amax)
        ctx.stride, ctx.pad, ctx.has_bias = stride, pad, b is not None
        ctx.side_ok = SIDE_OK[0]
        ctx.w_ref, ctx.b_ref = w, b
        ctx.save_for_backward(x, w4, col)
        return y

    @staticmethod
    def backward(ctx, dy):
        x, w4, col = ctx.saved_tensors
        dy = _c(dy)
        B_, H_, W_, Cin_ = x.shape
        Cout_, kh, kw, _ = w4.shape
        f16_d = ctx.needs_input_grad[0] and ops.conv3_f16_bwd_ok(B_, H_, W_, Cout_, Cin_, kh, kw, ctx.stride, ctx.pad)
        f16_w = col is None and ops.conv3_f16_wgrad_ok(B_, H_, W_, Cin_, Cout_, kh, kw, ctx.stride, ctx.pad)
        dy_amax = ops.amax(dy) if (f16_d or f16_w) else None
        if ctx.side_ok and ctx.needs_input_grad[0] and sinks(ctx.w_ref) and ops.conv_wgrad_stream_enabled(2, dy.numel() // dy.shape[-1]):
            cur, ws = torch.cuda.current_stream(dy.device), ops.side_stream(dy.device, "cwgrad")
            ws.wait_stream(cur)
            with torch.cuda.stream(ws):
                dw = _conv_wgrad_any(dy, x, col, tuple(w4.shape), ctx.stride, ctx.pad, ctx.w_ref, dy_amax=dy_amax, x_amax=ctx.x_amax)
                ops.reserve_for(ws, dy, x, col, dy_amax, ctx.x_amax)
            assert dw is None
        else:
            dw = _conv_wgrad_any(dy, x, col, tuple(w4.shape), ctx.stride, ctx.pad, ctx.w_ref, dy_amax=dy_amax, x_amax=ctx.x_amax)
        dx = ops.conv2d_dgrad(dy, w4, tuple(x.shape), ctx.stride, ctx.pad, dy_amax=dy_amax, w_owner=ctx.w_ref) if ctx.needs_input_grad[0] else None
        db = _bias_grad(ctx.b_ref, dy.view(-1, dy.shape[-1])) if ctx.has_bias else None
        return dx, dw, db, None, None


def _frozen_invstd(running_var, eps):
    tag = (running_var._version, ops.bn_epoch(), running_var.data_ptr(), float(eps))
    hit = running_var.__dict__.get("_vbg_invstd")
    if hit is not None and hit[0] == tag:
        return hit[1]
    with torch.no_grad():
        inv = torch.rsqrt(running_var + eps)
    running_var.__dict__["_vbg_invstd"] = (tag, inv)
    return inv


class ConvBnFn(torch.autograd.Function):

    @staticmethod
    def forward(ctx, x, w, gamma, beta, running_mean, running_var, res, stride, pad, relu, training, momentum, eps, sync):
        ctx.x_amax = _amax_tag(x)
        x = _c(x)
        sync = bool(sync) and SyncCtx.active()
        w4 = ohwi(w)
        fold = training and ops.bn_fold_ok(w.shape[0], sync)
        z, col, stats = _conv_any(x, w4, stride, pad, want_stats=training, w_owner=w, x_amax=ctx.x_amax, zero_slots=fold)
        C = z.shape[-1]
        z2 = z.view(-1, C)
        M = z2.shape[0]
        r2 = None if res is None else _c(res).view(-1, C)
        y_amax = ops.amax_slot(x.device) if (ops.conv3_f16_enabled() or (any(ctx.needs_input_grad) and ops.conv3_f16_bwd_enabled())) else None
        if fold:
            if stats is None:
                stats = ops.bn_stats(z2, ops.bn_zero_slots(x.device, C))
            count, count_dev = float(M), None
            y, mean, invstd = ops.bn_apply_fold(z2, r2, stats, count, eps, momentum, running_mean, running_var, gamma, beta, relu, y_amax=y_amax)
            y = y.view(z.shape)
        else:
            if training:
                if stats is None:
                    stats = ops.bn_stats(z2)
                count, count_dev = float(M), None
                if sync:
                    glob = ops.bn_fold_count(stats, C, M)
                    SyncCtx.all_reduce(glob)
                    count_dev = glob[2 * C:]
                    if ops.bn_fold_ok(C):
                        y, mean, invstd = ops.bn_apply_fold(z2, r2, glob, count, eps, momentum, running_mean, running_var, gamma, beta, relu,
                                                            y_amax=y_amax, nslots=1, count_dev=count_dev)
                        y = y.view(z.shape)
                    else:
                        mean, invstd = ops.bn_finalize(glob, C, 1, count, eps, momentum, running_mean, running_var, count_dev)
                else:
                    mean, invstd = ops.bn_finalize(stats, C, ops.bn_slots(), count, eps, momentum, running_mean, running_var)
            else:
                mean, invstd, count, count_dev = running_mean, _frozen_invstd(running_var, eps), float(M), None
            if not (training and sync and ops.bn_fold_ok(C)):
                y = ops.bn_apply(z2, r2, mean, invstd, gamma, beta, relu, y_amax=y_amax).view(z.shape)
        if y_amax is not None:
            y._vbg_amax = (y_amax, y._version)
        ctx.fold = fold
        ctx.side_ok = SIDE_OK[0]
        ctx.cfg = (stride, pad, relu, training, count, res is not None, sync)
        ctx.w_ref, ctx.affine = w, (gamma, beta)
        ctx.save_for_backward(x, w4, col, z, y if relu else None, mean, invstd, gamma, count_dev)
        return y

    @staticmethod
    def backward(ctx, dy):
        x, w4, col, z, y, mean, invstd, gamma, count_dev = ctx.saved_tensors
        stride, pad, relu, training, count, has_res, sync = ctx.cfg
        C = z.shape[-1]
        dy2 = _c(dy).view(-1, C)
        z2 = z.view(-1, C)
        y2 = None if y is None else y.view(-1, C)
        B_, H_, W_, Cin_ = x.shape
        want_amax = (ctx.needs_input_grad[0] and ops.conv3_f16_bwd_ok(B_, H_, W_, C, Cin_, w4.shape[1], w4.shape[2], stride, pad)) or \
            (col is None and ops.conv3_f16_wgrad_ok(B_, H_, W_, Cin_, C, w4.shape[1], w4.shape[2], stride, pad))
        dz_amax = ops.amax_slot(dy2.device) if want_amax else None
        dgamma, dbeta, sunk = _affine_dest(*ctx.affine)
        if ctx.fold and ops.bn_fold_ok(C, sync):
            slots = ops.bn_bwd_reduce(dy2, y2, z2, mean, invstd, relu, ops.bn_zero_slots(dy2.device, C))
            dz2, dres2 = ops.bn_bwd_apply_fold(dy2, y2, z2, mean, invstd, gamma, slots, count, relu, has_res, dgamma, dbeta, dx_amax=dz_amax)
            dgamma, dbeta = _affine_done(*ctx.affine, dgamma, dbeta, sunk)
            return ConvBnFn._finish_backward(ctx, dz2, dres2, dz_amax, dgamma, dbeta)
        slots = ops.bn_bwd_reduce(dy2, y2, z2, mean, invstd, relu)
        sums = ops.bn_param_grad(slots, C, dgamma, dbeta)
        dgamma, dbeta = _affine_done(*ctx.affine, dgamma, dbeta, sunk)
        if not training:
            sums = torch.zeros_like(sums)
        elif sync:
            SyncCtx.all_reduce(sums)
        dz2, dres2 = ops.bn_bwd_apply(dy2, y2, z2, mean, invstd, gamma, sums, count, relu, has_res, None, None, count_dev, dx_amax=dz_amax)
        return ConvBnFn._finish_backward(ctx, dz2, dres2, dz_amax, dgamma, dbeta)

    @staticmethod
    def _finish_backward(ctx, dz2, dres2, dz_amax, dgamma, dbeta):
        x, w4, col, z, y, mean, invstd, gamma, count_dev = ctx.saved_tensors
        stride, pad, relu, training, count, has_res, sync = ctx.cfg
        dz = dz2.view(z.shape)
        dres = dres2.view(z.shape) if has_res else None
        if ctx.side_ok and ctx.needs_input_grad[0] and sinks(ctx.w_ref) and ops.conv_wgrad_stream_enabled(1, dz2.shape[0]):
            cur, ws = torch.cuda.current_stream(dz.device), ops.side_stream(dz.device, "cwgrad")
            ws.wait_stream(cur)
            with torch.cuda.stream(ws):
                dw = _conv_wgrad_any(dz, x, col, tuple(w4.shape), stride, pad, ctx.w_ref, dy_amax=dz_amax, x_amax=ctx.x_amax)
                ops.reserve_for(ws, dz2, x, col, dz_amax, ctx.x_amax)
            assert dw is None
            dx = ops.conv2d_dgrad(dz, w4, tuple(x.shape), stride, pad, dy_amax=dz_amax, w_owner=ctx.w_ref)
            return dx, None, dgamma, dbeta, None, None, dres, None, None, None, None, None, None, None
        dx = ops.conv2d_dgrad(dz, w4, tuple(x.shape), stride, pad, dy_amax=dz_amax, w_owner=ctx.w_ref) if ctx.needs_input_grad[0] else None
        dw = _conv_wgrad_any(dz, x, col, tuple(w4.shape), stride, pad, ctx.w_ref, dy_amax=dz_amax, x_amax=ctx.x_amax)
        return dx, dw, dgamma, dbeta, None, None, dres, None, None, None, None, None, None, None


class MaxPoolFn(torch.autograd.Function):
    @staticmethod
    def forward(ctx, x):
        x = _c(x)
        y, am = ops.maxpool_fwd(x)
        ctx.hw = (x.shape[1], x.shape[2])
        ctx.save_for_backward(am)
        return y

    @staticmethod
    def backward(ctx, dy):
        (am,) = ctx.saved_tensors
        return ops.maxpool_bwd(_c(dy), am, *ctx.hw)


class AvgPool2Fn(torch.autograd.Function):

    @staticmethod
    def forward(ctx, x):
        x = _c(x)
        ctx.hw = (x.shape[1], x.shape[2])
        return ops.avgpool2_fwd(x)

    @staticmethod
    def backward(ctx, dy):
        return ops.avgpool2_bwd(_c(dy), *ctx.hw)


class UpAddFn(torch.autograd.Function):

    @staticmethod
    def forward(ctx, lo, skip):
        return ops.upsample2_add(_c(lo), _c(skip))

    @staticmethod
    def backward(ctx, dy):
        dy = _c(dy)
        return ops.sumpool(dy, 2), dy


class NhwcToNchwFlatFn(torch.autograd.Function):

    @staticmethod
    def forward(ctx, x):
        ctx.shape = x.shape
        return ops.nhwc_to_nchw(_c(x)).view(x.shape[0], -1)

    @staticmethod
    def backward(ctx, dy):
        N, h, w, C = ctx.shape
        return ops.nchw_to_nhwc(_c(dy).view(N, C, h, w))


class RoiAlignFn(torch.autograd.Function):
    @staticmethod
    def forward(ctx, feat, boxes, box_doc, out_size, scale):
        feat = _c(feat)
        ctx.cfg = (tuple(feat.shape), out_size, scale)
        ctx.save_for_backward(boxes, box_doc)
        return ops.roi_align_fwd(feat, boxes, box_doc, out_size, scale)

    @staticmethod
    def backward(ctx, dy):
        boxes, box_doc = ctx.saved_tensors
        shape, out_size, scale = ctx.cfg
        dfeat = torch.zeros(shape, device=dy.device, dtype=f32)
        ops.roi_align_bwd(_c(dy), shape, boxes, box_doc, out_size, scale, dfeat)
        return dfeat, None, None, None, None


class SegReduceFn(torch.autograd.Function):
    @staticmethod
    def forward(ctx, tok, tok_row, run_start, run_len, mode):
        tok = _c(tok)
        ctx.mode, ctx.shape = mode, tok.shape
        ctx.save_for_backward(tok_row, run_start, run_len)
        return ops.seg_reduce_fwd(tok, tok_row, run_start, run_len, mode)

    @staticmethod
# ... 637 lines not shown
```

### vibertgrid-pytorch_amd/vbg/lib.py

```python
import ctypes as C
import os

import torch

_HERE = os.path.dirname(os.path.abspath(__file__))
LIB_PATH = os.environ.get("VBG_LIB_PATH") or os.path.join(os.path.dirname(_HERE), "libvbg.so")

c_int, c_ll, c_f, c_d, c_vp, c_ull = C.c_int, C.c_longlong, C.c_float, C.c_double, C.c_void_p, C.c_ulonglong


class ConvGeo(C.Structure):
    _fields_ = [("Hs", c_int), ("Ws", c_int), ("Cs", c_int), ("Hr", c_int), ("Wr", c_int), ("kh", c_int), ("kw", c_int),
                ("stride", c_int), ("pad", c_int), ("dgrad", c_int)]


class GemmDesc(C.Structure):
    _fields_ = [("M", c_int), ("N", c_int), ("K", c_int),
                ("A", c_vp), ("lda", c_ll), ("a_kind", c_int), ("a_vec", c_int),
                ("a_nseg", c_int), ("a_seg_ptr", c_vp * 4), ("a_seg_kend", c_int * 4), ("a_seg_ld", c_ll * 4),
                ("a_seg_shift", c_int * 4), ("a_H", c_int), ("a_W", c_int),
                ("a_prologue", c_int), ("a_scale", c_f),
                ("B", c_vp), ("ldb", c_ll), ("b_kind", c_int), ("b_vec", c_int),
                ("geo", ConvGeo),
                ("C", c_vp), ("ldc", c_ll), ("C2", c_vp), ("bias", c_vp),
# ... 10 lines not shown
    _fields_ = [("A", c_vp), ("B", c_vp), ("C", c_vp), ("a_plane", c_ll), ("lda", c_ll), ("b_plane", c_ll), ("ldb", c_ll), ("ldc", c_ll),
                ("M", c_int), ("N", c_int), ("tiles_m", c_int), ("tiles_n", c_int), ("a_amax", c_vp)]


class PlaneGemmDesc(C.Structure):
    _fields_ = [("M", c_int), ("N", c_int), ("K", c_int),
                ("A", c_vp), ("a_plane", c_ll), ("lda", c_ll),
                ("B", c_vp), ("b_plane", c_ll), ("ldb", c_ll),
                ("C", c_vp), ("ldc", c_ll), ("C2", c_vp), ("bias", c_vp),
                ("Cp", c_vp), ("c_plane", c_ll), ("ldp", c_ll),
                ("epi", c_int), ("alpha", c_f), ("accumulate", c_int), ("splitk", c_int), ("tile", c_int), ("trans", c_int),
                ("ngroups", c_int), ("grp", PlaneGroup * 4),
                ("colsum", c_vp), ("form", c_int), ("Cq", c_vp), ("q_plane", c_ll), ("ldq", c_ll), ("a_amax", c_vp), ("c_amax", c_vp),
                ("cq_ref_in", c_vp), ("cq_l1_in", c_vp), ("cq_mul", c_f), ("cq_ref_out", c_vp)]


class L1Entry(C.Structure):
    _fields_ = [("w", c_vp), ("ld", c_ll), ("rows", c_int), ("cols", c_int)]


class AttnDesc(C.Structure):
    _fields_ = [("mode", c_int), ("heads", c_int), ("ntasks", c_int), ("max_len", c_int),
                ("tasks", c_vp), ("seq_len", c_vp), ("seq_row0", c_vp), ("pad_off", c_vp), ("ntok_pad", c_ll),
                ("qkv", c_vp), ("qkv_plane", c_ll), ("qkv_ld", c_ll),
                ("dO", c_vp), ("do_plane", c_ll), ("do_ld", c_ll),
                ("out", c_vp), ("ldo", c_ll), ("lse", c_vp), ("delta", c_vp), ("out_planes", c_vp), ("op_plane", c_ll), ("op_ld", c_ll), ("kbar", c_vp), ("ldk", c_ll), ("o", c_vp),
                ("mask_q", c_vp), ("mask_k", c_vp), ("mask_off", c_vp),
                ("scale", c_f), ("keep_scale", c_f), ("out_amax", c_vp), ("out_pair", c_vp), ("oq_plane", c_ll), ("oq_ld", c_ll),
                ("form", c_int), ("do_amax", c_vp)]


class PlanesRef(C.Structure):
    _fields_ = [("buf", c_vp), ("plane", c_ll), ("ld", c_ll)]


class BertLayerFwdDesc(C.Structure):
    _fields_ = [("ntok", c_int), ("hidden", c_int), ("inter", c_int), ("heads", c_int),
                ("eps", c_f), ("drop_p", c_f), ("seed", c_ull), ("stream_id0", c_ull),
                ("form_qkv", c_int), ("form_attn", c_int), ("form_ao", c_int), ("form_ffn", c_int),
                ("tile_qkv", c_int), ("tile_ao", c_int), ("tile_ffn1", c_int), ("tile_ffn2", c_int),
                ("ntasks", c_int), ("max_len", c_int), ("tasks", c_vp), ("seq_len", c_vp), ("seq_row0", c_vp), ("pad_off", c_vp), ("ntok_pad", c_ll),
                ("mask_q", c_vp), ("mask_k", c_vp), ("mask_off", c_vp), ("attn_scale", c_f), ("keep_scale", c_f),
                ("x", c_vp), ("xa", PlanesRef),
                ("wqkv", PlanesRef), ("wo", PlanesRef), ("wi", PlanesRef), ("wo2", PlanesRef),
                ("bqkv", c_vp), ("bo", c_vp), ("bi", c_vp), ("bo2", c_vp), ("g1", c_vp), ("b1", c_vp), ("g2", c_vp), ("b2", c_vp),
                ("pqkv", PlanesRef),
                ("ctx", c_vp), ("lse", c_vp), ("kbar", c_vp), ("pctx", PlanesRef), ("pctxq", PlanesRef),
                ("ao", c_vp), ("x1", c_vp), ("xhat1", c_vp), ("rstd1", c_vp), ("px1", PlanesRef), ("px1q", PlanesRef),
                ("h", c_vp), ("pg", PlanesRef), ("pgq", PlanesRef),
                ("fo", c_vp), ("y", c_vp), ("xhat2", c_vp), ("rstd2", c_vp), ("py", PlanesRef), ("pyq", PlanesRef)]


ATTN_FWD, ATTN_DQ, ATTN_DKV = 0, 1, 2
OP_DENSE_K, OP_DENSE_R, OP_CONV_K, OP_CONV_R, OP_WT_R = 0, 1, 2, 3, 4
EPI_NONE, EPI_RELU, EPI_GELU_DUAL, EPI_MUL_GELU_GRAD = 0, 1, 2, 3

SIGNATURES = {
    "vbg_version": (c_int, []),
    "vbg_gemm": (c_int, [C.POINTER(GemmDesc), c_vp]),
    "vbg_gemm_timed": (c_int, [C.POINTER(GemmDesc), c_vp, c_vp, c_vp]),
    "vbg_timer_create": (c_int, [c_vp]),
    "vbg_timer_destroy": (c_int, [c_vp]),
    "vbg_timer_elapsed_ms": (c_int, [c_vp, c_vp, c_vp]),
    "vbg_slab_reduce": (c_int, [c_vp, c_int, c_ll, c_int, c_int, c_ll, c_vp, c_int, c_vp, c_ll, c_vp]),
    "vbg_plane_gemm": (c_int, [C.POINTER(PlaneGemmDesc), c_vp]),
    "vbg_plane_gemm_timed": (c_int, [C.POINTER(PlaneGemmDesc), c_vp, c_vp, c_vp]),
    "vbg_split_planes": (c_int, [c_vp, c_ll, c_int, c_int, c_vp, c_int, c_ll, c_int, c_vp, c_vp]),
    "vbg_col_l1_max": (c_int, [c_vp, c_int, c_int, c_vp, c_vp]),
    "vbg_split_planes_pair": (c_int, [c_vp, c_ll, c_int, c_int, c_vp, c_int, c_ll, c_vp, c_vp, c_vp]),
    "vbg_split_planes_t": (c_int, [c_vp, c_ll, c_int, c_int, c_vp, c_int, c_ll, c_vp]),
    "vbg_split_planes_t_batched": (c_int, [c_vp, c_vp, c_vp, c_int, c_int, c_ll, c_vp]),
    "vbg_split_planes_pair_t_batched": (c_int, [c_vp, c_vp, c_vp, c_int, c_int, c_ll, c_vp]),
    "vbg_attn": (c_int, [C.POINTER(AttnDesc), c_vp]),
    "vbg_bert_layer_fwd": (c_int, [C.POINTER(BertLayerFwdDesc), c_vp]),
    "vbg_attn_drop_thr16": (C.c_uint, [c_f]),
    "vbg_attn_mask": (c_int, [c_vp, c_vp, c_int, c_int, c_int, c_f, c_ull, c_ull, c_vp, c_vp, c_vp]),
    "vbg_attn_mask_layers": (c_int, [c_vp, c_vp, c_int, c_int, c_int, c_f, c_ull, c_ull, c_ull, c_int, c_ll, c_vp, c_vp, c_vp]),
    "vbg_colsum": (c_int, [c_vp, c_ll, c_int, c_int, c_vp, c_int, c_vp]),
    "vbg_colsum_f64": (c_int, [c_vp, c_ll, c_int, c_int, c_vp, c_int, c_vp, c_vp]),
    "vbg_conv3x3": (c_int, [c_vp, c_vp, c_vp, c_vp, c_vp, c_int, c_int, c_int, c_int, c_int, c_int, c_int, c_int, c_vp, c_vp, c_vp, c_int, c_vp]),
    "vbg_conv3x3_split": (c_int, [c_int, c_int, c_int, c_int, c_int]),
    "vbg_conv3x3_pw": (c_int, [c_vp, c_vp, c_vp, c_vp, c_vp, c_int, c_int, c_int, c_int, c_int, c_int, c_int, c_vp, c_vp, c_vp, c_int, c_int, c_vp]),
    "vbg_conv3x3_pw_amp": (c_int, [c_vp, c_vp, c_vp, c_vp, c_vp, c_int, c_int, c_int, c_int, c_int, c_int, c_int, c_vp, c_vp, c_vp, c_int, c_int, c_vp]),
    "vbg_conv3x3_wprep": (c_int, [c_vp, c_vp, c_int, c_vp]),
    "vbg_conv3x3_wprep_bytes": (c_ll, [c_int, c_int, c_int, c_int]),
    "vbg_amax": (c_int, [c_vp, c_ll, c_vp, c_vp]),
    "vbg_conv3x3_wflip": (c_int, [c_vp, c_int, c_int, c_vp, c_vp]),
    "vbg_conv3x3_wgrad_strips": (c_int, [c_int, c_int, c_int, c_int, c_int]),
    "vbg_conv3x3_wgrad": (c_int, [c_vp, c_vp, c_vp, c_vp, c_int, c_int, c_int, c_int, c_int, c_int, c_vp, c_vp, c_vp]),
    "vbg_im2col": (c_int, [c_vp, c_int, c_int, c_int, c_int, c_int, c_int, c_int, c_int, c_int, c_vp, c_vp]),
    "vbg_normalize_resize": (c_int, [c_vp, c_int, c_int, c_int, c_int, C.POINTER(c_f), C.POINTER(c_f), c_vp, c_int, c_int, c_int, c_vp]),
    "vbg_rescale_boxes": (c_int, [c_vp, c_int, c_f, c_f, c_vp, c_vp]),
    "vbg_embed_ln_fwd": (c_int, [c_vp, c_vp, c_int, c_int, c_vp, c_vp, c_vp, c_vp, c_vp, c_f, c_f, c_ull, c_ull, c_vp, c_vp, c_vp, c_vp]),
    "vbg_embed_ln_bwd": (c_int, [c_vp, c_vp, c_vp, c_vp, c_vp, c_int, c_int, c_vp, c_f, c_ull, c_ull, c_vp, c_vp, c_vp, c_vp, c_vp, c_vp]),
    "vbg_dropout_add_ln_fwd": (c_int, [c_vp, c_vp, c_int, c_int, c_vp, c_vp, c_f, c_f, c_ull, c_ull, c_vp, c_vp, c_vp, c_vp]),
    "vbg_dropout_add_ln_fwd_planes": (c_int, [c_vp, c_vp, c_int, c_int, c_vp, c_vp, c_f, c_f, c_ull, c_ull, c_vp, c_vp, c_vp, c_vp, c_int, c_ll, c_vp, c_int, c_ll, c_vp]),
    "vbg_ln_bwd_ws_rows": (c_int, [c_int]),
    "vbg_dropout_add_ln_bwd": (c_int, [c_vp, c_vp, c_vp, c_int, c_int, c_vp, c_f, c_ull, c_ull, c_vp, c_vp, c_vp, c_vp, c_vp, c_vp, c_vp]),
    "vbg_dropout_add_ln_bwd_pair": (c_int, [c_vp, c_vp, c_vp, c_int, c_int, c_vp, c_f, c_ull, c_ull, c_vp, c_int, c_ll, c_vp, c_vp, c_vp, c_vp, c_vp, c_vp, c_vp, c_vp, c_vp]),
    "vbg_dropout_add_ln_bwd_planes": (c_int, [c_vp, c_vp, c_vp, c_int, c_int, c_vp, c_f, c_ull, c_ull, c_vp, c_int, c_ll, c_vp, c_vp, c_vp, c_vp, c_vp, c_vp]),
    "vbg_softmax_fwd": (c_int, [c_vp, c_vp, c_vp, c_vp, c_int, c_int, c_int, c_f, c_f, c_ull, c_ull, c_vp]),
    "vbg_softmax_bwd": (c_int, [c_vp, c_vp, c_vp, c_vp, c_vp, c_int, c_int, c_int, c_f, c_f, c_vp]),
    "vbg_row_softmax": (c_int, [c_vp, c_int, c_int, c_vp, c_vp]),
    "vbg_gelu_bwd": (c_int, [c_vp, c_vp, c_ll, c_vp]),
    "vbg_relu_bwd": (c_int, [c_vp, c_vp, c_ll, c_vp]),
    "vbg_add_inplace": (c_int, [c_vp, c_vp, c_ll, c_vp]),
    "vbg_scale_inplace": (c_int, [c_vp, c_ll, c_f, c_vp]),
    "vbg_seg_reduce_fwd": (c_int, [c_vp, c_vp, c_vp, c_vp, c_int, c_int, c_int, c_vp, c_vp]),
    "vbg_seg_reduce_bwd": (c_int, [c_vp, c_vp, c_vp, c_vp, c_int, c_int, c_int, c_vp, c_vp]),
    "vbg_owner_map": (c_int, [c_vp, c_vp, c_int, c_int, c_int, c_int, c_vp, c_vp]),
    "vbg_grid_scatter_fwd": (c_int, [c_vp, c_vp, c_int, c_int, c_int, c_int, c_int, c_vp, c_vp]),
    "vbg_grid_scatter_bwd": (c_int, [c_vp, c_vp, c_vp, c_vp, c_int, c_int, c_int, c_int, c_int, c_vp, c_vp]),
    "vbg_label_raster": (c_int, [c_vp, c_vp, c_ll, c_vp, c_vp, c_vp]),
    "vbg_bn_stats": (c_int, [c_vp, c_ll, c_int, c_vp, c_vp]),
    "vbg_bn_slots": (c_int, []),
    "vbg_bn_finalize": (c_int, [c_vp, c_int, c_int, c_d, c_vp, c_int, c_f, c_f, c_vp, c_vp, c_vp, c_vp, c_vp]),
    "vbg_bn_apply": (c_int, [c_vp, c_vp, c_ll, c_int, c_vp, c_vp, c_vp, c_vp, c_int, c_vp, c_vp, c_vp]),
    "vbg_bn_bwd_reduce": (c_int, [c_vp, c_vp, c_vp, c_ll, c_int, c_vp, c_vp, c_int, c_vp, c_vp]),
    "vbg_bn_bwd_apply": (c_int, [c_vp, c_vp, c_vp, c_ll, c_int, c_vp, c_vp, c_vp, c_vp, c_d, c_vp, c_int, c_vp, c_vp, c_vp, c_vp, c_vp, c_vp]),
    "vbg_bn_param_grad": (c_int, [c_vp, c_int, c_int, c_int, c_vp, c_vp, c_vp, c_vp]),
    "vbg_bn_apply_fold": (c_int, [c_vp, c_vp, c_ll, c_int, c_vp, c_int, c_d, c_vp, c_f, c_f, c_vp, c_vp, c_vp, c_vp, c_vp, c_vp, c_int, c_vp, c_vp, c_vp]),
    "vbg_bn_fold_count": (c_int, [c_vp, c_int, c_int, c_int, c_vp, c_d, c_vp]),
    "vbg_bn_bwd_apply_fold": (c_int, [c_vp, c_vp, c_vp, c_ll, c_int, c_vp, c_vp, c_vp, c_vp, c_int, c_d, c_int, c_vp, c_vp, c_vp, c_vp, c_vp, c_vp]),
    "vbg_maxpool3x3s2_fwd": (c_int, [c_vp, c_int, c_int, c_int, c_int, c_vp, c_vp, c_vp]),
    "vbg_maxpool3x3s2_bwd": (c_int, [c_vp, c_vp, c_int, c_int, c_int, c_int, c_int, c_int, c_vp, c_vp]),
    "vbg_avgpool2_fwd": (c_int, [c_vp, c_int, c_int, c_int, c_int, c_vp, c_vp]),
    "vbg_avgpool2_bwd": (c_int, [c_vp, c_int, c_int, c_int, c_int, c_vp, c_vp]),
    "vbg_upsample2_add": (c_int, [c_vp, c_vp, c_int, c_int, c_int, c_int, c_vp, c_vp]),
    "vbg_sumpool": (c_int, [c_vp, c_int, c_int, c_int, c_int, c_int, c_vp, c_int, c_vp]),
    "vbg_nchw_to_nhwc": (c_int, [c_vp, c_int, c_int, c_int, c_vp, c_vp]),
    "vbg_nhwc_to_nchw": (c_int, [c_vp, c_int, c_int, c_int, c_vp, c_vp]),
    "vbg_upsample_nhwc_to_nchw": (c_int, [c_vp, c_int, c_int, c_int, c_int, c_int, c_vp, c_vp]),
    "vbg_roi_align_fwd": (c_int, [c_vp, c_int, c_int, c_int, c_int, c_vp, c_vp, c_int, c_int, c_f, c_vp, c_vp]),
    "vbg_roi_align_bwd": (c_int, [c_vp, c_int, c_int, c_int, c_int, c_vp, c_vp, c_int, c_int, c_f, c_vp, c_vp]),
    "vbg_ce_fwd": (c_int, [c_vp, c_ll, c_int, c_vp, c_vp, c_ll, c_vp, c_int, c_int, c_int, c_vp, c_vp]),
    "vbg_ce_bwd": (c_int, [c_vp, c_ll, c_int, c_vp, c_vp, c_ll, c_vp, c_vp, c_f, c_int, c_int, c_int, c_vp, c_vp]),
    "vbg_compact_ws_bytes": (c_ll, [c_ll]),
    "vbg_compact": (c_int, [c_vp, c_ll, c_int, c_int, c_vp, c_vp, c_vp, c_ll, c_vp]),
    "vbg_sort_ws_bytes": (c_ll, [c_ll]),
    "vbg_sort_desc": (c_int, [c_vp, c_ll, c_vp, c_vp, c_vp, c_ll, c_vp]),
    "vbg_gather_f32": (c_int, [c_vp, c_vp, c_ll, c_vp, c_vp]),
    "vbg_gather_i32": (c_int, [c_vp, c_vp, c_ll, c_vp, c_vp]),
    "vbg_sum_f32": (c_int, [c_vp, c_ll, c_vp, c_vp]),
    "vbg_sumsq": (c_int, [c_vp, c_ll, c_vp, c_vp]),
    "vbg_gather_rows": (c_int, [c_vp, c_vp, c_ll, c_int, c_vp, c_vp]),
    "vbg_scatter_rows_add": (c_int, [c_vp, c_vp, c_ll, c_int, c_vp, c_vp]),
    "vbg_crf_nll_fwd": (c_int, [c_vp, c_vp, c_vp, c_int, c_vp, c_int, c_int, c_int, c_vp, c_vp, c_vp, c_vp]),
    "vbg_crf_nll_bwd": (c_int, [c_vp, c_vp, c_vp, c_int, c_vp, c_int, c_int, c_int, c_vp, c_vp, c_vp, c_vp, c_vp, c_vp]),
    "vbg_crf_viterbi": (c_int, [c_vp, c_vp, c_int, c_vp, c_int, c_int, c_int, c_vp, c_vp, c_vp, c_vp]),
    "vbg_sgd_step": (c_int, [c_vp, c_vp, c_vp, c_ll, c_f, c_f, c_f, c_int, c_f, c_vp]),
    "vbg_adamw_step": (c_int, [c_vp, c_vp, c_vp, c_vp, c_ll, c_f, c_f, c_f, c_f, c_f, c_int, c_f, c_vp]),
}


class VbgError(RuntimeError):
    pass


def _load():
    if not os.path.exists(LIB_PATH):
        raise ImportError(
            f"{LIB_PATH} not found: the HIP library is the product and there is no fallback. "
            "Build it with `make -C vibertgrid-pytorch_amd/csrc` (hipcc, gfx950).")
    lib = C.CDLL(LIB_PATH)
    for name, (res, args) in SIGNATURES.items():
        fn = getattr(lib, name)
        fn.restype = res
        fn.argtypes = args
    return lib


lib = _load()


def check(rc: int, what: str):
    if rc != 0:
        kind = "argument error" if rc < 0 else f"hipError {rc}"
        raise VbgError(f"{what} failed: {kind}")
```

### vibertgrid-pytorch_amd/vbg/ops.py

```python
import ctypes as C

import os

import torch

from .lib import (EPI_GELU_DUAL, EPI_NONE, EPI_RELU, OP_CONV_K, OP_CONV_R, OP_DENSE_K, OP_DENSE_R, OP_WT_R, ConvGeo,
                  AttnDesc, BertLayerFwdDesc, GemmDesc, PlaneGemmDesc, check, lib)

f32 = torch.float32
i32 = torch.int32


def raw_stream(device=None) -> int:
    idx = None if device is None else torch.device(device).index
    return torch._C._cuda_getCurrentRawStream(torch._C._cuda_getDevice() if idx is None else idx)


def _stream():
    return C.c_void_p(torch._C._cuda_getCurrentRawStream(torch._C._cuda_getDevice()))


_OVERLAP = [os.environ.get("VBG_OVERLAP", "1") != "0"]
_SIDE = {}


def overlap_enabled() -> bool:
    return _OVERLAP[0]


def set_overlap(on: bool):
    _OVERLAP[0] = bool(on)


_CONV_WGRAD_STREAM = [int(os.environ.get("VBG_CONV_WGRAD_STREAM", "2"))]


_CONV_WGRAD_STREAM_MAXPIX = [int(os.environ.get("VBG_CONV_WGRAD_STREAM_MAXPIX", "0"))]


def conv_wgrad_stream_enabled(level: int = 1, pixels: int = 0) -> bool:
    if _CONV_WGRAD_STREAM_MAXPIX[0] > 0 and pixels > _CONV_WGRAD_STREAM_MAXPIX[0]:
        return False
    return int(_CONV_WGRAD_STREAM[0]) >= level


_STAGE1_BWD_AFTER = [int(os.environ.get("VBG_STAGE1_BWD_AFTER", "6"))]


def stage1_bwd_after() -> int:
    return _STAGE1_BWD_AFTER[0]


def side_stream(device, name: str = "side") -> "torch.cuda.Stream":
    idx = torch.device(device).index
    if idx is None:
        idx = torch.cuda.current_device()
    s = _SIDE.get((idx, name))
    if s is None:
        s = _SIDE[(idx, name)] = torch.cuda.Stream(device=idx)
    return s


def reserve_for(stream, *tensors):
    for t in tensors:
        if t is not None:
            t.record_stream(stream)


def side_streams():
    return list(_SIDE.values())


def h2d(host, device):
    t = torch.from_numpy(host) if not torch.is_tensor(host) else host
    device = torch.device(device)
    if device.type != "cuda":
        return t.to(device)
    return t.pin_memory().to(device, non_blocking=True)


def _untag(t):
    if t is not None:
        t.__dict__.pop("_vbg_amax", None)


def P(t):
    if t is None:
        return None
    assert t.is_cuda, "libvbg operates on device memory only"
    return C.c_void_p(t.data_ptr())


def _vec_ok(t_ptr: int, ld: int) -> int:
    return int(t_ptr % 16 == 0 and ld % 4 == 0)


def _chk_f32(*ts):
    for t in ts:
        if t is not None:
            assert t.is_cuda and t.dtype == f32, (t.device, t.dtype)


_GEMM_F16 = [os.environ.get("VBG_GEMM_F16", "1") != "0"]


def set_gemm_f16(on: bool):
    _GEMM_F16[0] = bool(on)


def gemm_raw(M, N, K, A, lda, a_kind, B, ldb, b_kind, Cout, ldc, *, bias=None, epi=EPI_NONE, C2=None, accumulate=False,
             splitk=1, geo=None, segs=None, a_hw=(0, 0), a_relu_scale=None, grp=None, ngroups=0, grp_max=(0, 0), tile=0,
             alpha=1.0, a_ptr_off=0, b_ptr_off=0, c_ptr_off=0, bk=0, stats=None, slab_stride=0, f16=False):
    d = GemmDesc()
    d.M, d.N, d.K = int(M), int(N), int(K)
    ap = A.data_ptr() + 4 * a_ptr_off
    bp = B.data_ptr() + 4 * b_ptr_off
    d.A, d.lda, d.a_kind = ap, int(lda), a_kind
    d.B, d.ldb, d.b_kind = bp, int(ldb), b_kind
    d.a_vec = _vec_ok(ap, lda)
    d.b_vec = _vec_ok(bp, ldb)
    if segs:
        d.a_nseg = len(segs)
        vec = 1
        for i, (t, kend, ld, sh) in enumerate(segs):
            d.a_seg_ptr[i] = t.data_ptr()
            d.a_seg_kend[i] = int(kend)
            d.a_seg_ld[i] = int(ld)
            d.a_seg_shift[i] = int(sh)
            vec &= _vec_ok(t.data_ptr(), ld)
        d.a_vec = vec
        d.a_H, d.a_W = int(a_hw[0]), int(a_hw[1])
    if a_relu_scale is not None:
        d.a_prologue, d.a_scale = 1, float(a_relu_scale)
    if geo is not None:
        d.geo = geo
    d.C, d.ldc = Cout.data_ptr() + 4 * c_ptr_off, int(ldc)
    d.C2 = None if C2 is None else C2.data_ptr() + 4 * c_ptr_off
    d.bias = None if bias is None else bias.data_ptr()
    if stats is not None:
        d.stats, d.stats_slots = stats.data_ptr(), bn_slots()
    if splitk == 1 and not accumulate and torch.is_grad_enabled() and stats is None:
        splitk = 0
    if splitk == 0 and accumulate:
        splitk = 1
    if accumulate:
        _untag(Cout)
    d.epi, d.alpha, d.accumulate, d.splitk, d.tile = epi, float(alpha), int(bool(accumulate)), int(splitk), int(tile)
    d.bk = int(bk)
    d.slab_stride = int(slab_stride)
    if _AMP[0] or _SPLIT3[0]:
        d.bf16 = 1 if _AMP[0] else (2 if (f16 and _GEMM_F16[0] and grp is None) else 3)
        if _DISPATCH[0] is not None and not _AMP[0] and grp is None:
            _seen("gemm:f16x2" if d.bf16 == 2 else "gemm:bf16x3")
        if bk == 16:
            d.bk = 0
        if grp is not None and not _AMP[0]:
            d.bf16, d.bk = 0, int(bk)
    if _FORCE[0] or _FORCE[1]:
        d.tile, d.bk = _FORCE[0] or d.tile, _FORCE[1] or d.bk
    if grp is not None:
        d.grp, d.ngroups = grp.data_ptr(), int(ngroups)
        d.grp_maxM, d.grp_maxN = int(grp_max[0]), int(grp_max[1])
    prof = _GEMM_PROF
    if prof is not None and prof.match(a_kind, b_kind, grp is not None):
        e0, e1 = prof.events()
        check(lib.vbg_gemm_timed(C.byref(d), _stream(), e0, e1), "vbg_gemm_timed")
# ... 394 lines not shown
    M, N = dy.shape
    K = w.shape[1]
    assert w.shape[0] == N and dy.stride(1) == 1 and w.stride(1) == 1
    if out is None:
        assert not accumulate
        out = torch.empty((M, K), device=dy.device, dtype=f32)
    gemm_raw(M, K, N, dy, dy.stride(0), OP_DENSE_K, w, w.stride(0), OP_DENSE_R, out, out.stride(0), accumulate=accumulate, splitk=_BWD_SPLIT)
    return out


def linear_wgrad(dy, x, out, accumulate=True):
    _chk_f32(dy, x, out)
    M, N = dy.shape
    K = x.shape[1]
    assert x.shape[0] == M and out.shape == (N, K) and dy.stride(1) == 1 and x.stride(1) == 1
    sk = _pick_splitk(N, K, M)
    if not accumulate and sk > 1:
        out.zero_()
    gemm_raw(N, K, M, dy, dy.stride(0), OP_DENSE_R, x, x.stride(0), OP_DENSE_R, out, out.stride(0),
             accumulate=(accumulate or sk > 1), splitk=sk)
    return out


def colsum(x, out=None, accumulate=False):
    _chk_f32(x)
    M, N = x.shape
    assert x.stride(1) == 1
    if out is None:
        out = torch.empty((N,), device=x.device, dtype=f32)
        accumulate = False
    key = (x.device, raw_stream(x.device))
    ws = _COLSUM_WS.get(key)
    if ws is None or ws.numel() < N:
        ws = _COLSUM_WS[key] = torch.empty((max(N, 4096),), device=x.device, dtype=torch.float64)
    check(lib.vbg_colsum_f64(P(x), x.stride(0), M, N, P(out), int(accumulate), P(ws), _stream()), "vbg_colsum_f64")
    return out


_COLSUM_WS = {}


def conv_geo(Hs, Ws, Cs, Hr, Wr, kh, kw, stride, pad, dgrad=0):
    g = ConvGeo()
    g.Hs, g.Ws, g.Cs, g.Hr, g.Wr, g.kh, g.kw, g.stride, g.pad, g.dgrad = Hs, Ws, Cs, Hr, Wr, kh, kw, stride, pad, dgrad
    return g


def conv_out_hw(H, W, k, stride, pad):
    return (H + 2 * pad - k) // stride + 1, (W + 2 * pad - k) // stride + 1


def fuse_stats_ok(M, N, K):
    tiles = ((M + 63) // 64) * ((N + 63) // 64)
    return N % 4 == 0 and not (tiles <= 384 and (K + 31) // 32 >= 48)


_CONV3 = [os.environ.get("VBG_CONV3", "1") != "0"]


def set_conv3(on: bool):
    _CONV3[0] = bool(on)


_CONV3_MIN_TILES = [int(os.environ.get("VBG_CONV3_MIN_TILES", "480"))]
_CONV3_MIN_TILES_FWD = [int(os.environ.get("VBG_CONV3_MIN_TILES_FWD", "256"))]


def conv3_ok(B, H, W, Cs, N, kh, kw, stride, pad, fwd=False) -> bool:
    if not (_CONV3[0] and _SPLIT3[0] and not _amp_generic() and kh == 3 and kw == 3 and stride == 1 and pad == 1 and Cs % 16 == 0):
        return False
    min_tiles = _CONV3_MIN_TILES_FWD[0] if fwd and _CONV3_F16[0] else _conv3_min_tiles_bwd()
    if H == 7 and W == 7:
        return N % 128 == 0 and B * 49 * Cs < (1 << 29) and ((B + 1) // 2) * 2 * (N // 128) >= min_tiles
    if not (W in (16, 32, 64, 128, 256, 512, 1024) and (H * W) % 64 == 0 and H * W * Cs < (1 << 29)):
        return False
    if N % 128 == 0:
        return (B * H * W // 64) * (N // 128) >= min_tiles or conv3_split(B, H, W, Cs, N) > 1
    if N % 64 == 0:
        return (H * W) % 128 == 0 and (B * H * W // 128) * (N // 64) >= 240
    return False


_CONV3_F16 = [os.environ.get("VBG_CONV3_F16", "1") != "0"]
_CONV3_MIN_TILES_BWD = [int(os.environ.get("VBG_CONV3_MIN_TILES_BWD", "0"))]


def _conv3_min_tiles_bwd():
    if _CONV3_MIN_TILES_BWD[0] > 0:
        return _CONV3_MIN_TILES_BWD[0]
    return _CONV3_MIN_TILES[0]


def conv3_f16_enabled() -> bool:
    return _CONV3_F16[0] and _CONV3[0] and _SPLIT3[0]


def set_conv3_f16(on: bool):
    _CONV3_F16[0] = bool(on)


_AMAX_POOL = {}
_AMAX_POOL_SLOTS = [int(os.environ.get("VBG_AMAX_POOL_SLOTS", "256"))]


AMAX_WORDS, AMAX_STRIDE = 64, 32


def amax_slot(device):
    key = (device.type, device.index, raw_stream(device) if device.type == "cuda" else 0)
    ent = _AMAX_POOL.get(key)
    if ent is None or ent[1] >= ent[0].shape[0]:
        ent = _AMAX_POOL[key] = [torch.zeros((_AMAX_POOL_SLOTS[0], AMAX_WORDS * AMAX_STRIDE), device=device, dtype=torch.int32), 0]
    i = ent[1]
    ent[1] = i + 1
    return ent[0][i]


def amax(x, slot=None):
    slot = amax_slot(x.device) if slot is None else slot
    check(lib.vbg_amax(P(x), x.numel(), P(slot), _stream()), "vbg_amax")
    return slot


_CONV3_SPLITK = [os.environ.get("VBG_CONV3_SPLITK", "1") != "0"]
_CONV3_TICKETS = {}


def conv3_split(B, H, W, Cs, N) -> int:
    return int(lib.vbg_conv3x3_split(B, H, W, Cs, N)) if _CONV3_SPLITK[0] else 1


def _conv3_tickets(device, tiles):
    key = (device.index, torch.cuda.current_stream(device).cuda_stream)
    t = _CONV3_TICKETS.get(key)
    if t is None or t.numel() < tiles:
        t = _CONV3_TICKETS[key] = torch.zeros(max(1024, tiles), device=device, dtype=torch.int32)
    return t


def conv3x3(x, w_ohwi, bias=None, out=None, stats=None, accumulate=False, f16x2=False, x_amax=None, nsplit=None, w_planes=None, n_out=None, bn=0):
    B, H, W, Cs = x.shape
    N = w_ohwi.shape[0] if n_out is None else int(n_out)
    if out is None:
        assert not accumulate
        out = torch.empty((B, H, W, N), device=x.device, dtype=f32)
    elif accumulate:
        _untag(out)
    assert x_amax is None or f16x2
    assert w_planes is None or f16x2
    nz = conv3_split(B, H, W, Cs, N) if nsplit is None else int(nsplit)
    slab = tickets = None
    if nz > 1:
        tiles = (B * H * W // 128) * (N // (bn or 128))
        slab = torch.empty((tiles * nz, 128 * (bn or 128)), device=x.device, dtype=f32)
        tickets = _conv3_tickets(x.device, tiles)
    if _DISPATCH[0] is not None:
        _seen("conv3:fwd")
        if nz > 1:
            _seen("conv3:split")
        if H == 7 and W == 7:
            _seen("conv3:roi")
        if f16x2:
            _seen("conv3:f16x2")
        if bn == 64:
            _seen("conv3:bn64")
    ev = None
    if _CONV3_PROF[0] is not None:
        ev = (torch.cuda.Event(enable_timing=True), torch.cuda.Event(enable_timing=True))
        ev[0].record()
    if w_planes is not None:
        _seen("conv3:pw")
        onep = _AMP[0] and _AMP_FAST[0]
        if onep:
            _seen("conv3:onep")
        check((lib.vbg_conv3x3_pw_amp if onep else lib.vbg_conv3x3_pw)(P(x), P(w_planes), P(bias), P(out), P(stats), bn_slots() if stats is not None else 0,
                                                                     B, H, W, Cs, N, int(accumulate), P(x_amax), P(slab), P(tickets), nz, int(bn), _stream()),
              "vbg_conv3x3_pw")
    else:
        check(lib.vbg_conv3x3(P(x), P(w_ohwi), P(bias), P(out), P(stats), bn_slots() if stats is not None else 0, B, H, W, Cs, N,
                              int(accumulate), int(bool(f16x2)), P(x_amax), P(slab), P(tickets), nz, _stream()), "vbg_conv3x3")
    if ev is not None:
        ev[1].record()
        _CONV3_PROF[0].append((2.0 * B * H * W * Cs * N * 9, (1 if (w_planes is not None and _AMP[0] and _AMP_FAST[0]) else 3) if f16x2 else 6, ev[0], ev[1]))
    return out


_CONV3_PROF = [None]
_DISPATCH = [None]


def dispatch_log(on: bool):
    _DISPATCH[0] = {} if on else None
    return _DISPATCH[0]


def _seen(key):
    d = _DISPATCH[0]
    if d is not None:
        d[key] = d.get(key, 0) + 1


def set_conv3_profiler(records):
    _CONV3_PROF[0] = records


_WL1 = {"entries": [], "table": None, "host": None, "out": None, "maxc": 0}


def weight_col_l1max(owner, view=None):
    from .lib import L1Entry
    import weakref
    w = owner if view is None else view
    assert w.dim() == 2 and w.stride(1) == 1
    st = _WL1
    slot = owner.__dict__.get("_vbg_l1")
    tag = (_W_EPOCH[0], owner._version, w.data_ptr())
    if slot is not None and slot["tag"] == tag:
        return st["out"][slot["idx"]:slot["idx"] + 1]
    if slot is None or slot["ptr"] != w.data_ptr():
        st["entries"] = [e for e in st["entries"] if e["ref"]() is not owner]
        slot = {"idx": -1, "tag": None, "ptr": w.data_ptr(), "shape": tuple(w.shape), "ld": w.stride(0), "ref": weakref.ref(owner)}
        owner.__dict__["_vbg_l1"] = slot
        st["entries"].append(slot)
        st["table"] = None
    keep = []
    for e in st["entries"]:
        o = e["ref"]()
        if o is not None and (e is slot or o.data_ptr() == e["ptr"]):
            keep.append(e)
        elif o is not None:
            o.__dict__.pop("_vbg_l1", None)
    if len(keep) != len(st["entries"]):
        st["entries"] = keep
        st["table"] = None
    if st["table"] is None or st["out"] is None or st["table"].device != w.device:
        n = len(st["entries"])
        host = (L1Entry * n)()
        for i, e in enumerate(st["entries"]):
            e["idx"] = i
            host[i].w, host[i].ld, host[i].rows, host[i].cols = e["ptr"], e["ld"], e["shape"][0], e["shape"][1]
        st["host"] = host
        st["table"] = h2d(torch.frombuffer(bytearray(bytes(host)), dtype=torch.uint8), w.device)
        st["out"] = torch.zeros((max(n, 64),), device=w.device, dtype=torch.int32)
        st["maxc"] = max(e["shape"][1] for e in st["entries"])
    else:
        st["out"].zero_()
    check(lib.vbg_col_l1_max(P(st["table"]), len(st["entries"]), st["maxc"], P(st["out"]), _stream()), "vbg_col_l1_max")
    for e in st["entries"]:
        o = e["ref"]()
        if o is not None:
            e["tag"] = (_W_EPOCH[0], o._version, e["ptr"])
    return st["out"][slot["idx"]:slot["idx"] + 1]


_C3PW = {"entries": [], "table": None, "host": None, "n": 0}


# ... 87 lines not shown

def conv3x3_wgrad(dy, x, dw_ohwi, slabs=True, f16x2=False, dy_amax=None, x_amax=None):
    B, H, W, Cs = x.shape
    Cout = dy.shape[3]
    slab = None
    if slabs:
        strips = int(lib.vbg_conv3x3_wgrad_strips(B, H, W, Cs, Cout))
        slab = torch.empty((strips, dw_ohwi.numel()), device=x.device, dtype=f32)
    if f16x2:
        dy_amax = amax(dy) if dy_amax is None else dy_amax
        x_amax = amax(x) if x_amax is None else x_amax
    _seen("conv3:wgrad")
    form = (2 if (_AMP[0] and _AMP_FAST[0]) else 1) if f16x2 else 0
    if form == 2:
        _seen("conv3:wgrad_onep")
    check(lib.vbg_conv3x3_wgrad(P(dy), P(x), P(dw_ohwi), P(slab), B, H, W, Cs, Cout, form, P(dy_amax), P(x_amax), _stream()),
          "vbg_conv3x3_wgrad")
    return dw_ohwi


def conv2d_fwd(x, w_ohwi, stride, pad, bias=None, out=None, stats=None, w_owner=None, x_amax=None):
    _chk_f32(x, w_ohwi, bias)
    B, H, W, Cin = x.shape
    Cout, kh, kw, _ = w_ohwi.shape
    assert x.is_contiguous() and w_ohwi.is_contiguous() and w_ohwi.shape[3] == Cin and Cin % 16 == 0
    Ho, Wo = conv_out_hw(H, W, kh, stride, pad)
    if out is None:
        out = torch.empty((B, Ho, Wo, Cout), device=x.device, dtype=f32)
    M, K = B * Ho * Wo, kh * kw * Cin
    if conv3_ok(B, H, W, Cin, Cout, kh, kw, stride, pad, fwd=True):
        late = conv3_late_choice(B, H, W, Cin, Cout) if _CONV3_F16[0] else None
        if late is not None:
            wp = conv3_planes(w_owner, w_ohwi, False, bn=late[0])
            if wp is not None:
                return conv3x3(x, w_ohwi, bias, out, stats, f16x2=True, w_planes=wp, x_amax=x_amax, nsplit=late[1], bn=late[0])
        wp = conv3_planes(w_owner, w_ohwi, False) if (_CONV3_F16[0] and conv3_pw_ok(B, H, W, Cin, Cout)) else None
        return conv3x3(x, w_ohwi, bias, out, stats, f16x2=_CONV3_F16[0], w_planes=wp, x_amax=x_amax if _CONV3_F16[0] else None)
    if kh == 1 and kw == 1 and stride == 1 and pad == 0:
        gemm_raw(M, Cout, K, x, Cin, OP_DENSE_K, w_ohwi, K, OP_DENSE_K, out, Cout, bias=bias, stats=stats, f16=True)
    else:
        gemm_raw(M, Cout, K, x, Cin, OP_CONV_K, w_ohwi, K, OP_DENSE_K, out, Cout, bias=bias,
                 geo=conv_geo(H, W, Cin, Ho, Wo, kh, kw, stride, pad, 0), stats=stats, f16=True)
    return out


_BWD_SPLIT = 0


def conv3_f16_bwd_enabled() -> bool:
    return _CONV3[0] and _SPLIT3[0] and not _amp_generic() and _CONV3_F16[0]


def conv3_f16_bwd_ok(B, H, W, Cout, Cin, kh, kw, stride, pad) -> bool:
    return _CONV3_F16[0] and conv3_ok(B, H, W, Cout, Cin, kh, kw, stride, pad)


def conv3_late_choice(B, H, W, Cs, N):
    if not _CONV3_SPLITK[0] or (H == 7 and W == 7) or N % 128 or (H * W) % 128 or W >= 128 or Cs % 16:
        return None
    t128 = (B * H * W // 128) * (N // 128)
    if t128 >= 240 or t128 < 4:
        return None
    t64 = 2 * t128
    nz = 1 if t64 >= 240 else min(4, -(-480 // t64))
    while nz > 1:
        cs = nz // 3 if nz % 3 == 0 else nz
        if Cs % cs == 0 and (Cs // cs) % 16 == 0:
            break
        nz -= 1
    return 64, nz


def conv3_pw_ok(B, H, W, Cs, N) -> bool:
    if H == 7 and W == 7:
        return True
    if (H * W) % 128 != 0:
        return False
    if conv3_split(B, H, W, Cs, N) > 1 or W >= 128:
        return True
    bn = 64 if (N % 128 != 0 and N % 64 == 0) else 128
    return (B * H * W // 128) * ((N + bn - 1) // bn) >= 240


def conv2d_dgrad(dy, w_ohwi, x_shape, stride, pad, out=None, accumulate=False, dy_amax=None, w_owner=None):
    _chk_f32(dy, w_ohwi)
    B, H, W, Cin = x_shape
    Cout, kh, kw, _ = w_ohwi.shape
    Bq, Ho, Wo, Cq = dy.shape
    assert dy.is_contiguous() and w_ohwi.is_contiguous() and Cq == Cout and Bq == B
    if out is None:
        assert not accumulate
        out = torch.empty(x_shape, device=dy.device, dtype=f32)
    M = B * H * W
    if conv3_ok(B, H, W, Cout, Cin, kh, kw, stride, pad):
        if _CONV3_F16[0]:
            late = conv3_late_choice(B, H, W, Cout, Cin)
            if late is not None:
                wp = conv3_planes(w_owner, w_ohwi, True, bn=late[0])
                if wp is not None:
                    return conv3x3(dy, w_ohwi, None, out, None, accumulate, f16x2=True, x_amax=dy_amax if dy_amax is not None else amax(dy),
                                   w_planes=wp, n_out=Cin, nsplit=late[1], bn=late[0])
            wp = conv3_planes(w_owner, w_ohwi, True) if conv3_pw_ok(B, H, W, Cout, Cin) else None
            if wp is not None:
                return conv3x3(dy, w_ohwi, None, out, None, accumulate, f16x2=True, x_amax=dy_amax if dy_amax is not None else amax(dy),
                               w_planes=wp, n_out=Cin)
            return conv3x3(dy, conv3x3_wflip(w_ohwi), None, out, None, accumulate, f16x2=True, x_amax=dy_amax if dy_amax is not None else amax(dy))
        return conv3x3(dy, conv3x3_wflip(w_ohwi), None, out, None, accumulate)
    if kh == 1 and kw == 1 and stride == 1 and pad == 0:
        gemm_raw(M, Cin, Cout, dy, Cout, OP_DENSE_K, w_ohwi, Cin, OP_DENSE_R, out, Cin, accumulate=accumulate, splitk=_BWD_SPLIT)
    else:
        assert Cout % 16 == 0 and Cin % 4 == 0
        gemm_raw(M, Cin, kh * kw * Cout, dy, Cout, OP_CONV_K, w_ohwi, Cin, OP_WT_R, out, Cin, accumulate=accumulate,
                 geo=conv_geo(Ho, Wo, Cout, H, W, kh, kw, stride, pad, 1), splitk=_BWD_SPLIT)
    return out


def conv3_f16_wgrad_ok(B, H, W, Cin, Cout, kh, kw, stride, pad) -> bool:
    return _CONV3_F16[0] and conv3w_ok(B, H, W, Cin, Cout, kh, kw, stride, pad)


def conv2d_wgrad(dy, x, dw_ohwi, stride, pad, accumulate=True, dy_amax=None, x_amax=None):
    _chk_f32(dy, x, dw_ohwi)
    B, H, W, Cin = x.shape
    Cout, kh, kw, _ = dw_ohwi.shape
    _, Ho, Wo, _ = dy.shape
    assert dy.is_contiguous() and x.is_contiguous() and dw_ohwi.is_contiguous()
    Mpix, Kc = B * Ho * Wo, kh * kw * Cin
    if conv3w_ok(B, H, W, Cin, Cout, kh, kw, stride, pad):
        if not accumulate:
            dw_ohwi.zero_()
        if _CONV3_F16[0]:
            return conv3x3_wgrad(dy, x, dw_ohwi, f16x2=True, dy_amax=dy_amax, x_amax=x_amax)
        return conv3x3_wgrad(dy, x, dw_ohwi)
    sk = _pick_splitk(Cout, Kc, Mpix)
    if not accumulate and sk > 1:
        dw_ohwi.zero_()
    acc = accumulate or sk > 1
    if kh == 1 and kw == 1 and stride == 1 and pad == 0:
        gemm_raw(Cout, Kc, Mpix, dy, Cout, OP_DENSE_R, x, Cin, OP_DENSE_R, dw_ohwi, Kc, accumulate=acc, splitk=sk)
    else:
        assert Cin % 16 == 0
        gemm_raw(Cout, Kc, Mpix, dy, Cout, OP_DENSE_R, x, Cin, OP_CONV_R, dw_ohwi, Kc, accumulate=acc, splitk=sk,
                 geo=conv_geo(H, W, Cin, Ho, Wo, kh, kw, stride, pad, 0))
    return dw_ohwi


def im2col(x, kh, kw, stride, pad, Kpad):
    _chk_f32(x)
    B, H, W, Cc = x.shape
    Ho, Wo = conv_out_hw(H, W, kh, stride, pad)
    out = torch.empty((B * Ho * Wo, Kpad), device=x.device, dtype=f32)
    check(lib.vbg_im2col(P(x), B, H, W, Cc, kh, kw, stride, pad, Kpad, P(out), _stream()), "vbg_im2col")
    return out


def embed_ln_fwd(ids, pos_ids, word, pos, type0, gamma, beta, eps, p, seed, sid):
    ntok, hidden = ids.numel(), word.shape[1]
    out = torch.empty((ntok, hidden), device=word.device, dtype=f32)
    xhat = torch.empty_like(out)
    rstd = torch.empty((ntok,), device=word.device, dtype=f32)
    check(lib.vbg_embed_ln_fwd(P(ids), P(pos_ids), ntok, hidden, P(word), P(pos), P(type0), P(gamma), P(beta), eps, p, seed, sid,
                               P(out), P(xhat), P(rstd), _stream()), "vbg_embed_ln_fwd")
    return out, xhat, rstd


def embed_ln_bwd(dout, xhat, rstd, ids, pos_ids, gamma, p, seed, sid, dword, dpos, dtype0, dgamma, dbeta):
    ntok, hidden = xhat.shape
    check(lib.vbg_embed_ln_bwd(P(dout), P(xhat), P(rstd), P(ids), P(pos_ids), ntok, hidden, P(gamma), p, seed, sid, P(dword),
                               P(dpos), P(dtype0), P(dgamma), P(dbeta), _stream()), "vbg_embed_ln_bwd")


def dropout_add_ln_fwd(x, res, gamma, beta, eps, p, seed, sid, out_planes=None, out_pair=None):
    rows, hidden = x.shape
    y = torch.empty_like(x)
    xhat = torch.empty_like(x)
    rstd = torch.empty((rows,), device=x.device, dtype=f32)
    if out_planes is not None or out_pair is not None:
        assert (out_planes is None or (out_planes.ld == hidden and out_planes.rows == rows)) and (out_pair is None or out_pair.ld == hidden)
        check(lib.vbg_dropout_add_ln_fwd_planes(P(x), P(res), rows, hidden, P(gamma), P(beta), eps, p, seed, sid, P(y), P(xhat), P(rstd),
                                                P(out_planes.buf) if out_planes is not None else None, out_planes.ld if out_planes is not None else 0,
                                                out_planes.plane if out_planes is not None else 0,
                                                P(out_pair.buf) if out_pair is not None else None, out_pair.ld if out_pair is not None else 0,
                                                out_pair.plane if out_pair is not None else 0, _stream()), "vbg_dropout_add_ln_fwd_planes")
        return y, xhat, rstd
    check(lib.vbg_dropout_add_ln_fwd(P(x), P(res), rows, hidden, P(gamma), P(beta), eps, p, seed, sid, P(y), P(xhat), P(rstd),
                                     _stream()), "vbg_dropout_add_ln_fwd")
    return y, xhat, rstd


_LN_WS = {}
# ... 294 lines not shown
def bn_fold_ok(C_, sync=False) -> bool:
    return not sync and C_ % 64 == 0


def bn_zero_slots(device, C_):
    key = (device, raw_stream(device))
    n = bn_slots() * 2 * C_
    ent = _BN_ZPOOL.get(key)
    if ent is None or ent[1] + n > ent[0].numel():
        ent = _BN_ZPOOL[key] = [torch.zeros((max(1 << 20, n),), device=device, dtype=torch.float64), 0]
    o = ent[1]
    ent[1] = o + n
    return ent[0][o:o + n]


def bn_fold_count(slots, C_, count):
    out = torch.empty((2 * C_ + 1,), device=slots.device, dtype=torch.float64)
    check(lib.vbg_bn_fold_count(P(slots), bn_slots(), 1, C_, P(out), float(count), _stream()), "vbg_bn_fold_count")
    return out


def bn_apply_fold(x2d, res2d, slots, count, eps, momentum, running_mean, running_var, gamma, beta, relu, y_amax=None, nslots=None, count_dev=None):
    M, C_ = x2d.shape
    out = torch.empty_like(x2d)
    mean = torch.empty((C_,), device=x2d.device, dtype=f32)
    invstd = torch.empty_like(mean)
    check(lib.vbg_bn_apply_fold(P(x2d), P(res2d), M, C_, P(slots), bn_slots() if nslots is None else int(nslots), float(count), P(count_dev), eps, momentum,
                                P(mean), P(invstd), P(running_mean), P(running_var), P(gamma), P(beta), int(relu), P(out), P(y_amax), _stream()),
          "vbg_bn_apply_fold")
    if running_var is not None:
        _BN_EPOCH[0] += 1
    return out, mean, invstd


def bn_bwd_apply_fold(dy, y, x, mean, invstd, gamma, slots, count, relu, want_dres, dgamma, dbeta, dx_amax=None):
    M, C_ = x.shape
    dx = torch.empty_like(x)
    dres = torch.empty_like(x) if want_dres else None
    check(lib.vbg_bn_bwd_apply_fold(P(dy), P(y), P(x), M, C_, P(mean), P(invstd), P(gamma), P(slots), bn_slots(), float(count), int(relu), P(dx),
                                    P(dres), P(dgamma), P(dbeta), P(dx_amax), _stream()), "vbg_bn_bwd_apply_fold")
    return dx, dres


def bn_stats(x2d, stats=None):
    M, C_ = x2d.shape
    if stats is None:
        stats = _bn_workspace(x2d.device, C_)
    check(lib.vbg_bn_stats(P(x2d), M, C_, P(stats), _stream()), "vbg_bn_stats")
    return stats


def bn_fold(slots, C_, out=None):
    if out is None:
        out = torch.empty((2 * C_,), device=slots.device, dtype=torch.float64)
    check(lib.vbg_bn_param_grad(P(slots), bn_slots(), 1, C_, P(out), None, None, _stream()), "vbg_bn_param_grad")
    return out


def bn_finalize(stats, C_, nslots, count, eps, momentum, running_mean, running_var, count_dev=None):
    mean = torch.empty((C_,), device=stats.device, dtype=f32)
    invstd = torch.empty_like(mean)
    check(lib.vbg_bn_finalize(P(stats), int(nslots), int(nslots > 1), float(count), P(count_dev), C_, eps, momentum, P(mean), P(invstd),
                              P(running_mean), P(running_var), _stream()), "vbg_bn_finalize")
    if running_var is not None:
        _BN_EPOCH[0] += 1
    return mean, invstd


_BN_EPOCH = [0]


def bn_epoch() -> int:
    return _BN_EPOCH[0]


def bn_apply(x2d, res2d, mean, invstd, gamma, beta, relu, out=None, y_amax=None):
    M, C_ = x2d.shape
    if out is None:
        out = torch.empty_like(x2d)
    check(lib.vbg_bn_apply(P(x2d), P(res2d), M, C_, P(mean), P(invstd), P(gamma), P(beta), int(relu), P(out), P(y_amax), _stream()), "vbg_bn_apply")
    return out


def bn_bwd_reduce(dy, y, x, mean, invstd, relu, sums=None):
    M, C_ = x.shape
    if sums is None:
        sums = _bn_workspace(x.device, C_)
    check(lib.vbg_bn_bwd_reduce(P(dy), P(y), P(x), M, C_, P(mean), P(invstd), int(relu), P(sums), _stream()), "vbg_bn_bwd_reduce")
    return sums


def bn_bwd_apply(dy, y, x, mean, invstd, gamma, sums, count, relu, want_dres, dgamma, dbeta, count_dev=None, dx_amax=None):
    M, C_ = x.shape
    dx = torch.empty_like(x)
    dres = torch.empty_like(x) if want_dres else None
    check(lib.vbg_bn_bwd_apply(P(dy), P(y), P(x), M, C_, P(mean), P(invstd), P(gamma), P(sums), float(count), P(count_dev), int(relu), P(dx), P(dres),
                               P(dgamma), P(dbeta), P(dx_amax), _stream()), "vbg_bn_bwd_apply")
    return dx, dres


def bn_param_grad(slots, C_, dgamma, dbeta):
    folded = torch.empty((2 * C_,), device=slots.device, dtype=torch.float64)
    check(lib.vbg_bn_param_grad(P(slots), bn_slots(), 1, C_, P(folded), P(dgamma), P(dbeta), _stream()), "vbg_bn_param_grad")
    return folded


def maxpool_fwd(x):
    B, H, W, C_ = x.shape
    Ho, Wo = conv_out_hw(H, W, 3, 2, 1)
    y = torch.empty((B, Ho, Wo, C_), device=x.device, dtype=f32)
    am = torch.empty((B, Ho, Wo, C_), device=x.device, dtype=i32)
    check(lib.vbg_maxpool3x3s2_fwd(P(x), B, H, W, C_, P(y), P(am), _stream()), "vbg_maxpool_fwd")
    return y, am


def maxpool_bwd(dy, am, H, W):
    B, Ho, Wo, C_ = dy.shape
    dx = torch.empty((B, H, W, C_), device=dy.device, dtype=f32)
    check(lib.vbg_maxpool3x3s2_bwd(P(dy), P(am), B, Ho, Wo, C_, H, W, P(dx), _stream()), "vbg_maxpool_bwd")
    return dx


def avgpool2_fwd(x):
    B, H, W, C_ = x.shape
    y = torch.empty((B, H // 2, W // 2, C_), device=x.device, dtype=f32)
    check(lib.vbg_avgpool2_fwd(P(x), B, H, W, C_, P(y), _stream()), "vbg_avgpool2_fwd")
    return y


def avgpool2_bwd(dy, H, W):
    B, _, _, C_ = dy.shape
    dx = torch.empty((B, H, W, C_), device=dy.device, dtype=f32)
    check(lib.vbg_avgpool2_bwd(P(dy), B, H, W, C_, P(dx), _stream()), "vbg_avgpool2_bwd")
    return dx


def upsample2_add(lo, skip):
    B, H, W, C_ = skip.shape
    y = torch.empty_like(skip)
    check(lib.vbg_upsample2_add(P(lo), P(skip), B, H, W, C_, P(y), _stream()), "vbg_upsample2_add")
    return y


def sumpool(hi, f, out=None, accumulate=False):
    B, H, W, C_ = hi.shape
    if out is None:
        out = torch.empty((B, H // f, W // f, C_), device=hi.device, dtype=f32)
        accumulate = False
    elif accumulate:
        _untag(out)
    check(lib.vbg_sumpool(P(hi), B, H, W, C_, f, P(out), int(accumulate), _stream()), "vbg_sumpool")
    return out


def nchw_to_nhwc(x):
    B, C_, H, W = x.shape
    y = torch.empty((B, H, W, C_), device=x.device, dtype=f32)
    check(lib.vbg_nchw_to_nhwc(P(x), B, C_, H * W, P(y), _stream()), "vbg_nchw_to_nhwc")
    return y


def nhwc_to_nchw(x):
    B, H, W, C_ = x.shape
    y = torch.empty((B, C_, H, W), device=x.device, dtype=f32)
    check(lib.vbg_nhwc_to_nchw(P(x), B, C_, H * W, P(y), _stream()), "vbg_nhwc_to_nchw")
    return y


def upsample_nhwc_to_nchw(x, f):
    B, h, w, C_ = x.shape
# ... 139 lines not shown
```

Before: 270.2.

## Fuse BN backward reduction and ReLU mask into conv3x3 dgrad epilogue

The conv3x3 dgrad kernel epilogue now takes the following BN layer's pre-activation z and affine parameters. It recomputes the ReLU mask and accumulates the BN backward sums (masked dy and dy*xhat) directly into stats slots. That removes the separate bn_bwd_reduce pass over dy, y and z. The BN backward apply then uses a new z-masked variant that recomputes the mask from z instead of reading y. In exchange the epilogue carries extra register pressure from z prefetch and per-channel parameter loads, and the Python side needs tensor tagging to pass the BN source through autograd.

Result: no change. 270.4, median of 6 (+0.1%).

```diff
diff --git a/include/vbg.h b/include/vbg.h
--- a/include/vbg.h
+++ b/include/vbg.h
@@ -146,6 +146,9 @@
 int vbg_conv3x3_pw_amp(const float* x, const void* w_planes, const float* bias, float* y, double* stats, int stats_slots, int B, int H, int W,
                        int Cs, int N, int accumulate, const unsigned* x_amax, float* split_slab, unsigned* split_tickets, int nsplit,
                        int bn, void* stream);
+int vbg_conv3x3_bn_bwd(const float* dy, const float* w, const void* w_planes, float* dx, double* sums, int sums_slots, int B, int H, int W,
+                       int Cs, int N, int form, const unsigned* dy_amax, float* split_slab, unsigned* split_tickets, int nsplit, int bn,
+                       const float* z, const float* mean, const float* invstd, const float* gamma, const float* beta, void* stream);
 
 int vbg_conv3x3_wgrad_strips(int B, int H, int W, int Cs, int Cout);
 int vbg_conv3x3_wgrad(const float* dy, const float* x, float* dw, float* slab, int B, int H, int W, int Cs, int Cout, int form,
@@ -245,6 +248,9 @@
 int vbg_bn_bwd_apply_fold(const float* dy, const float* y, const float* x, long long M, int C, const float* mean,
                           const float* invstd, const float* gamma, double* slots, int nslots, double count, int relu, float* dx,
                           float* dres, float* dgamma_accum, float* dbeta_accum, unsigned* dx_amax, void* stream);
+int vbg_bn_bwd_apply_fold_z(const float* dy, const float* z, long long M, int C, const float* mean, const float* invstd, const float* gamma,
+                            const float* beta, double* slots, int nslots, double count, float* dx, float* dgamma_accum, float* dbeta_accum,
+                            unsigned* dx_amax, void* stream);
 int vbg_bn_param_grad(double* slots, int nslots, int clear_slots, int C, double* folded, float* dgamma_accum, float* dbeta_accum,
                       void* stream);
 int vbg_maxpool3x3s2_fwd(const float* x, int B, int H, int W, int C, float* y, int* argmax, void* stream);
diff --git a/vibertgrid-pytorch_amd/csrc/conv3.hip b/vibertgrid-pytorch_amd/csrc/conv3.hip
--- a/vibertgrid-pytorch_amd/csrc/conv3.hip
+++ b/vibertgrid-pytorch_amd/csrc/conv3.hip
@@ -24,6 +24,11 @@
     unsigned* tickets;
     int accumulate;
     const unsigned* a_amax;
+    const float* bn_z;
+    const float* bn_mean;
+    const float* bn_invstd;
+    const float* bn_gamma;
+    const float* bn_beta;
 };
 
 __device__ __forceinline__ __amdgpu_buffer_rsrc_t c3_rsrc(const float* base) {
@@ -453,8 +458,27 @@
             for (int r = 0; r < 16; ++r)
                 Ct[(wm * (BM / 2) + i * 32 + (r & 3) + 8 * (r >> 2) + 4 * lk) * CTS + wn * (BN / 2) + j * 32 + lr] =
                     ONEP ? acc[i][j][r] * a_sc.y : (F16 ? (acc[i][j][r] + acx[i][j][r] * (1.f / 2048.f)) * a_sc.y : acc[i][j][r]);
+    constexpr int QN = BN / 4;
+    constexpr int NEP = BM * QN / NT;
+    const float* const bn_z = p.bn_z;
+    const int egn = n0 + (tid % QN) * 4;
+    float4 zpre[NEP];
+    auto z_prefetch = [&]() {
+#pragma unroll
+        for (int q = 0; q < NEP; ++q) {
+            const int row = (tid + q * NT) / QN;
+            int gm = m0 + row;
+            bool ok = egn < N;
+            if (roi) {
+                const int im = nb + (row >> 6), sy = (row >> 3) & 7, sx = row & 7;
+                ok = ok && !(im >= roi || sy == 7 || sx == 7);
+                gm = im * 49 + sy * 7 + sx;
+            }
+            zpre[q] = ok ? *reinterpret_cast<const float4*>(bn_z + (long long)gm * N + egn) : make_float4(0.f, 0.f, 0.f, 0.f);
+        }
+    };
+    if (bn_z && nz == 1) z_prefetch();
     __syncthreads();
-    constexpr int QN = BN / 4;
     const float* part = nullptr;
     if (nz > 1) {
         unsigned& ticket_s = smem[SMEM];
@@ -479,10 +503,16 @@
         }
         __syncthreads();
         part = p.slab + tile * nz * (size_t)(BM * BN);
+        if (bn_z) z_prefetch();
     }
     float4 cs = make_float4(0.f, 0.f, 0.f, 0.f), cq = cs;
-#pragma unroll 4
-    for (int q = 0; q < BM * QN / NT; ++q) {
+    float4 bmu = cs, bis = cs, bga = cs, bbe = cs;
+    if (bn_z && egn < N) {
+        bmu = *reinterpret_cast<const float4*>(p.bn_mean + egn); bis = *reinterpret_cast<const float4*>(p.bn_invstd + egn);
+        bga = *reinterpret_cast<const float4*>(p.bn_gamma + egn); bbe = *reinterpret_cast<const float4*>(p.bn_beta + egn);
+    }
+#pragma unroll
+    for (int q = 0; q < NEP; ++q) {
         const int idx = tid + q * NT;
         const int row = idx / QN, c = (idx % QN) * 4;
         int gm = m0 + row;
@@ -505,7 +535,16 @@
         }
         if (bias) { v.x += bias[gn]; v.y += bias[gn + 1]; v.z += bias[gn + 2]; v.w += bias[gn + 3]; }
         float* cp = p.Y + (long long)gm * N + gn;
-        if (p.stats) {
+        if (bn_z) {
+            const float4 zv = zpre[q];
+            const float gx = bn_affine(zv.x, bmu.x, bis.x, bga.x, bbe.x) > 0.f ? v.x : 0.f;
+            const float gy = bn_affine(zv.y, bmu.y, bis.y, bga.y, bbe.y) > 0.f ? v.y : 0.f;
+            const float gz = bn_affine(zv.z, bmu.z, bis.z, bga.z, bbe.z) > 0.f ? v.z : 0.f;
+            const float gw = bn_affine(zv.w, bmu.w, bis.w, bga.w, bbe.w) > 0.f ? v.w : 0.f;
+            cs.x += gx; cs.y += gy; cs.z += gz; cs.w += gw;
+            cq.x += gx * ((zv.x - bmu.x) * bis.x); cq.y += gy * ((zv.y - bmu.y) * bis.y);
+            cq.z += gz * ((zv.z - bmu.z) * bis.z); cq.w += gw * ((zv.w - bmu.w) * bis.w);
+        } else if (p.stats) {
             cs.x += v.x; cs.y += v.y; cs.z += v.z; cs.w += v.w;
             cq.x += v.x * v.x; cq.y += v.y * v.y; cq.z += v.z * v.z; cq.w += v.w * v.w;
         }
@@ -941,9 +980,12 @@
     VBG_LAUNCH_RET();
 }
 
+struct conv3_bn_src {
+    const float *z, *mean, *invstd, *gamma, *beta;
+};
 static int conv3x3_impl(const float* x, const float* w, const unsigned short* wp, const float* bias, float* y, double* stats, int stats_slots,
                         int B, int H, int W, int Cs, int N, int accumulate, int form, const unsigned* x_amax, float* split_slab,
-                        unsigned* split_tickets, int nsplit, void* stream, int bn_req = 0);
+                        unsigned* split_tickets, int nsplit, void* stream, int bn_req = 0, const conv3_bn_src* bns = nullptr);
 
 extern "C" int vbg_conv3x3(const float* x, const float* w, const float* bias, float* y, double* stats, int stats_slots, int B, int H,
                            int W, int Cs, int N, int accumulate, int form, const unsigned* x_amax, float* split_slab,
@@ -968,9 +1010,23 @@
                         split_tickets, nsplit, stream, bn);
 }
 
+extern "C" int vbg_conv3x3_bn_bwd(const float* dy, const float* w, const void* w_planes, float* dx, double* sums, int sums_slots, int B, int H,
+                                  int W, int Cs, int N, int form, const unsigned* dy_amax, float* split_slab, unsigned* split_tickets,
+                                  int nsplit, int bn, const float* z, const float* mean, const float* invstd, const float* gamma,
+                                  const float* beta, void* stream) {
+    VBG_CHECK_ARG(sums && sums_slots >= 1 && z && mean && invstd && gamma && beta && (w != nullptr) != (w_planes != nullptr));
+    VBG_CHECK_ARG((((uintptr_t)z) & 15) == 0 && (((uintptr_t)mean) & 15) == 0 && (((uintptr_t)invstd) & 15) == 0 &&
+                  (((uintptr_t)gamma) & 15) == 0 && (((uintptr_t)beta) & 15) == 0);
+    VBG_CHECK_ARG(!w_planes || ((((uintptr_t)w_planes) & 15) == 0 && form >= 1 && (bn == 0 || bn == 64 || bn == 128)));
+    VBG_CHECK_ARG(w_planes || (form <= 1 && bn == 0));
+    const conv3_bn_src bns = {z, mean, invstd, gamma, beta};
+    return conv3x3_impl(dy, w, (const unsigned short*)w_planes, nullptr, dx, sums, sums_slots, B, H, W, Cs, N, 0, form, dy_amax, split_slab,
+                        split_tickets, nsplit, stream, bn, &bns);
+}
+
 static int conv3x3_impl(const float* x, const float* w, const unsigned short* wp, const float* bias, float* y, double* stats, int stats_slots,
                         int B, int H, int W, int Cs, int N, int accumulate, int form, const unsigned* x_amax, float* split_slab,
-                        unsigned* split_tickets, int nsplit, void* stream, int bn_req) {
+                        unsigned* split_tickets, int nsplit, void* stream, int bn_req, const conv3_bn_src* bns) {
     VBG_CHECK_ARG(form == 0 || form == 1 || (form == 2 && wp));
     VBG_CHECK_ARG(bn_req == 0 || wp);
     VBG_CHECK_ARG(!x_amax || form >= 1);
@@ -984,6 +1040,8 @@
     VBG_CHECK_ARG(!stats || (stats_slots >= 1 && !accumulate));
     vbg::conv3_args a;
     a.X = x; a.Wt = w; a.Wp = wp; a.bias = bias; a.Y = y; a.stats = stats; a.stats_slots = stats_slots;
+    a.bn_z = bns ? bns->z : nullptr; a.bn_mean = bns ? bns->mean : nullptr; a.bn_invstd = bns ? bns->invstd : nullptr;
+    a.bn_gamma = bns ? bns->gamma : nullptr; a.bn_beta = bns ? bns->beta : nullptr;
     a.H = H; a.W = W; a.wsh = roi ? 3 : 31 - __builtin_clz((unsigned)W); a.Cs = Cs; a.N = N;
     const long long M = (long long)B * H * W;
     VBG_CHECK_ARG(M < (1ll << 31));
diff --git a/vibertgrid-pytorch_amd/csrc/convaux.hip b/vibertgrid-pytorch_amd/csrc/convaux.hip
--- a/vibertgrid-pytorch_amd/csrc/convaux.hip
+++ b/vibertgrid-pytorch_amd/csrc/convaux.hip
@@ -234,8 +234,8 @@
         const long long i = r * C4 + cq;
         const float4 xv = reinterpret_cast<const float4*>(x)[i];
         float4 o;
-        o.x = (xv.x - mu.x) * is.x * ga.x + be.x; o.y = (xv.y - mu.y) * is.y * ga.y + be.y;
-        o.z = (xv.z - mu.z) * is.z * ga.z + be.z; o.w = (xv.w - mu.w) * is.w * ga.w + be.w;
+        o.x = bn_affine(xv.x, mu.x, is.x, ga.x, be.x); o.y = bn_affine(xv.y, mu.y, is.y, ga.y, be.y);
+        o.z = bn_affine(xv.z, mu.z, is.z, ga.z, be.z); o.w = bn_affine(xv.w, mu.w, is.w, ga.w, be.w);
         if (res) {
             const float4 rv = reinterpret_cast<const float4*>(res)[i];
             o.x += rv.x; o.y += rv.y; o.z += rv.z; o.w += rv.w;
@@ -247,14 +247,16 @@
     if (amax) amax_publish_at(mx, amax, blockIdx.x + blockIdx.y * gridDim.x);
 }
 
+template <bool ZMASK>
 __global__ __launch_bounds__(256) void bn_bwd_apply_fold_kernel(const float* __restrict__ dy, const float* __restrict__ y,
                                                                 const float* __restrict__ x, long long M, int C,
                                                                 const float* __restrict__ mean, const float* __restrict__ invstd,
                                                                 const float* __restrict__ gamma, double* __restrict__ slots, int nslots,
                                                                 double count, int relu, int rows_per_block, float* __restrict__ dx,
-                                                                float* __restrict__ dres, float* dgamma, float* dbeta, unsigned* amax) {
+                                                                float* __restrict__ dres, float* dgamma, float* dbeta, unsigned* amax,
+                                                                const float* __restrict__ beta) {
     __shared__ double fold[128];
-    __shared__ __attribute__((aligned(16))) float cst[5][64];
+    __shared__ __attribute__((aligned(16))) float cst[ZMASK ? 6 : 5][64];
     const int tid = threadIdx.x, c0 = blockIdx.y * 64;
     if (tid < 128) fold[tid] = fold_slots(slots, nslots, C, (tid >> 6) * C + c0 + (tid & 63), false);
     __syncthreads();
@@ -264,6 +266,7 @@
         const double sg = fold[tid], sgx = fold[64 + tid];
         cst[0][tid] = mean[c]; cst[1][tid] = invstd[c]; cst[2][tid] = gamma[c];
         cst[3][tid] = (float)sg * icnt; cst[4][tid] = (float)sgx * icnt;
+        if constexpr (ZMASK) cst[5][tid] = beta[c];
         if (blockIdx.x == 0) {
             if (dbeta) dbeta[c] += (float)sg;
             if (dgamma) dgamma[c] += (float)sgx;
@@ -274,17 +277,22 @@
     const float4 mu = reinterpret_cast<const float4*>(cst[0])[q], is = reinterpret_cast<const float4*>(cst[1])[q];
     const float4 ga = reinterpret_cast<const float4*>(cst[2])[q], s0 = reinterpret_cast<const float4*>(cst[3])[q];
     const float4 s1 = reinterpret_cast<const float4*>(cst[4])[q];
+    float4 be = s1;
+    if constexpr (ZMASK) be = reinterpret_cast<const float4*>(cst[ZMASK ? 5 : 4])[q];
     const long long r0 = (long long)blockIdx.x * rows_per_block, r1 = min(M, r0 + rows_per_block);
     float mx = 0.f;
 #pragma unroll 4
     for (long long r = r0 + rl; r < r1; r += 16) {
         const long long i = r * C4 + cq;
         float4 g = reinterpret_cast<const float4*>(dy)[i];
-        if (relu) {
+        const float4 xv = reinterpret_cast<const float4*>(x)[i];
+        if constexpr (ZMASK) {
+            g.x = bn_affine(xv.x, mu.x, is.x, ga.x, be.x) > 0.f ? g.x : 0.f; g.y = bn_affine(xv.y, mu.y, is.y, ga.y, be.y) > 0.f ? g.y : 0.f;
+            g.z = bn_affine(xv.z, mu.z, is.z, ga.z, be.z) > 0.f ? g.z : 0.f; g.w = bn_affine(xv.w, mu.w, is.w, ga.w, be.w) > 0.f ? g.w : 0.f;
+        } else if (relu) {
             const float4 yv = reinterpret_cast<const float4*>(y)[i];
             g.x = yv.x > 0.f ? g.x : 0.f; g.y = yv.y > 0.f ? g.y : 0.f; g.z = yv.z > 0.f ? g.z : 0.f; g.w = yv.w > 0.f ? g.w : 0.f;
         }
-        const float4 xv = reinterpret_cast<const float4*>(x)[i];
         float4 o;
         o.x = ga.x * is.x * (g.x - s0.x - (xv.x - mu.x) * is.x * s1.x);
         o.y = ga.y * is.y * (g.y - s0.y - (xv.y - mu.y) * is.y * s1.y);
@@ -631,8 +639,19 @@
     VBG_CHECK_ARG(((dgamma_accum == nullptr) == (dbeta_accum == nullptr)) && ALIGNED16(dy) && ALIGNED16(x) && ALIGNED16(dx) &&
                   (!relu || ALIGNED16(y)) && (!dres || ALIGNED16(dres)));
     const int rpb = bn_fold_rows(M, C);
-    VBG_LAUNCH(bn_bwd_apply_fold_kernel, dim3(cdiv(M, rpb), C / 64), dim3(256), 0, S_, dy, y, x, M, C, mean, invstd, gamma, slots, nslots, count,
-               relu, rpb, dx, dres, dgamma_accum, dbeta_accum, dx_amax);
+    VBG_LAUNCH(bn_bwd_apply_fold_kernel<false>, dim3(cdiv(M, rpb), C / 64), dim3(256), 0, S_, dy, y, x, M, C, mean, invstd, gamma, slots, nslots,
+               count, relu, rpb, dx, dres, dgamma_accum, dbeta_accum, dx_amax, (const float*)nullptr);
+    VBG_LAUNCH_RET();
+}
+
+extern "C" int vbg_bn_bwd_apply_fold_z(const float* dy, const float* z, long long M, int C, const float* mean, const float* invstd,
+                                       const float* gamma, const float* beta, double* slots, int nslots, double count, float* dx,
+                                       float* dgamma_accum, float* dbeta_accum, unsigned* dx_amax, void* stream) {
+    VBG_CHECK_ARG(dy && z && mean && invstd && gamma && beta && slots && dx && M > 0 && C > 0 && C % 64 == 0 && nslots >= 1 && count > 0);
+    VBG_CHECK_ARG(((dgamma_accum == nullptr) == (dbeta_accum == nullptr)) && ALIGNED16(dy) && ALIGNED16(z) && ALIGNED16(dx));
+    const int rpb = bn_fold_rows(M, C);
+    VBG_LAUNCH(bn_bwd_apply_fold_kernel<true>, dim3(cdiv(M, rpb), C / 64), dim3(256), 0, S_, dy, (const float*)nullptr, z, M, C, mean, invstd, gamma,
+               slots, nslots, count, 1, rpb, dx, (float*)nullptr, dgamma_accum, dbeta_accum, dx_amax, beta);
     VBG_LAUNCH_RET();
 }
 
diff --git a/vibertgrid-pytorch_amd/csrc/vbg_common.h b/vibertgrid-pytorch_amd/csrc/vbg_common.h
--- a/vibertgrid-pytorch_amd/csrc/vbg_common.h
+++ b/vibertgrid-pytorch_amd/csrc/vbg_common.h
@@ -89,6 +89,7 @@
     const float pdf = 0.39894228040143267794f * __expf(-0.5f * x * x);
     return cdf + x * pdf;
 }
+__device__ __forceinline__ float bn_affine(float z, float mu, float is, float ga, float be) { return (z - mu) * is * ga + be; }
 
 }
 
diff --git a/vibertgrid-pytorch_amd/vbg/functions.py b/vibertgrid-pytorch_amd/vbg/functions.py
--- a/vibertgrid-pytorch_amd/vbg/functions.py
+++ b/vibertgrid-pytorch_amd/vbg/functions.py
@@ -72,6 +72,13 @@
         return None
     slot, version = tag
     return slot if x._version == version else None
+
+
+def _bn_src_tag(x):
+    tag = getattr(x, "_vbg_bn_src", None)
+    if tag is None:
+        return None
+    return tag[0] if x._version == tag[1] else None
 
 
 class SyncCtx:
@@ -316,6 +323,7 @@
     @staticmethod
     def forward(ctx, x, w, gamma, beta, running_mean, running_var, res, stride, pad, relu, training, momentum, eps, sync):
         ctx.x_amax = _amax_tag(x)
+        ctx.x_bn = _bn_src_tag(x)
         x = _c(x)
         sync = bool(sync) and SyncCtx.active()
         w4 = ohwi(w)
@@ -355,6 +363,8 @@
                 y = ops.bn_apply(z2, r2, mean, invstd, gamma, beta, relu, y_amax=y_amax).view(z.shape)
         if y_amax is not None:
             y._vbg_amax = (y_amax, y._version)
+        if fold and relu and res is None and gamma is not None and beta is not None and ops.bn_fuse_enabled():
+            y._vbg_bn_src = ((z2, mean, invstd, gamma, beta), y._version)
         ctx.fold = fold
         ctx.side_ok = SIDE_OK[0]
         ctx.cfg = (stride, pad, relu, training, count, res is not None, sync)
@@ -376,7 +386,14 @@
         dz_amax = ops.amax_slot(dy2.device) if want_amax else None
         dgamma, dbeta, sunk = _affine_dest(*ctx.affine)
         if ctx.fold and ops.bn_fold_ok(C, sync):
-            slots = ops.bn_bwd_reduce(dy2, y2, z2, mean, invstd, relu, ops.bn_zero_slots(dy2.device, C))
+            slots = ops.bn_sums_tag(dy, z2) if relu else None
+            if slots is None:
+                slots = ops.bn_bwd_reduce(dy2, y2, z2, mean, invstd, relu, ops.bn_zero_slots(dy2.device, C))
+            beta = ctx.affine[1]
+            if relu and not has_res and beta is not None and ops.bn_fuse_enabled():
+                dz2 = ops.bn_bwd_apply_fold_z(dy2, z2, mean, invstd, gamma, beta, slots, count, dgamma, dbeta, dx_amax=dz_amax)
+                dgamma, dbeta = _affine_done(*ctx.affine, dgamma, dbeta, sunk)
+                return ConvBnFn._finish_backward(ctx, dz2, None, dz_amax, dgamma, dbeta)
             dz2, dres2 = ops.bn_bwd_apply_fold(dy2, y2, z2, mean, invstd, gamma, slots, count, relu, has_res, dgamma, dbeta, dx_amax=dz_amax)
             dgamma, dbeta = _affine_done(*ctx.affine, dgamma, dbeta, sunk)
             return ConvBnFn._finish_backward(ctx, dz2, dres2, dz_amax, dgamma, dbeta)
@@ -403,9 +420,12 @@
                 dw = _conv_wgrad_any(dz, x, col, tuple(w4.shape), stride, pad, ctx.w_ref, dy_amax=dz_amax, x_amax=ctx.x_amax)
                 ops.reserve_for(ws, dz2, x, col, dz_amax, ctx.x_amax)
             assert dw is None
-            dx = ops.conv2d_dgrad(dz, w4, tuple(x.shape), stride, pad, dy_amax=dz_amax, w_owner=ctx.w_ref)
+            dx = ops.conv2d_dgrad(dz, w4, tuple(x.shape), stride, pad, dy_amax=dz_amax, w_owner=ctx.w_ref, bn_src=ctx.x_bn)
+            ctx.x_bn = None
             return dx, None, dgamma, dbeta, None, None, dres, None, None, None, None, None, None, None
-        dx = ops.conv2d_dgrad(dz, w4, tuple(x.shape), stride, pad, dy_amax=dz_amax, w_owner=ctx.w_ref) if ctx.needs_input_grad[0] else None
+        dx = ops.conv2d_dgrad(dz, w4, tuple(x.shape), stride, pad, dy_amax=dz_amax, w_owner=ctx.w_ref, bn_src=ctx.x_bn) \
+            if ctx.needs_input_grad[0] else None
+        ctx.x_bn = None
         dw = _conv_wgrad_any(dz, x, col, tuple(w4.shape), stride, pad, ctx.w_ref, dy_amax=dz_amax, x_amax=ctx.x_amax)
         return dx, dw, dgamma, dbeta, None, None, dres, None, None, None, None, None, None, None
 
diff --git a/vibertgrid-pytorch_amd/vbg/lib.py b/vibertgrid-pytorch_amd/vbg/lib.py
--- a/vibertgrid-pytorch_amd/vbg/lib.py
+++ b/vibertgrid-pytorch_amd/vbg/lib.py
@@ -116,6 +116,8 @@
     "vbg_conv3x3_split": (c_int, [c_int, c_int, c_int, c_int, c_int]),
     "vbg_conv3x3_pw": (c_int, [c_vp, c_vp, c_vp, c_vp, c_vp, c_int, c_int, c_int, c_int, c_int, c_int, c_int, c_vp, c_vp, c_vp, c_int, c_int, c_vp]),
     "vbg_conv3x3_pw_amp": (c_int, [c_vp, c_vp, c_vp, c_vp, c_vp, c_int, c_int, c_int, c_int, c_int, c_int, c_int, c_vp, c_vp, c_vp, c_int, c_int, c_vp]),
+    "vbg_conv3x3_bn_bwd": (c_int, [c_vp, c_vp, c_vp, c_vp, c_vp, c_int, c_int, c_int, c_int, c_int, c_int, c_int, c_vp, c_vp, c_vp, c_int, c_int,
+                                   c_vp, c_vp, c_vp, c_vp, c_vp, c_vp]),
     "vbg_conv3x3_wprep": (c_int, [c_vp, c_vp, c_int, c_vp]),
     "vbg_conv3x3_wprep_bytes": (c_ll, [c_int, c_int, c_int, c_int]),
     "vbg_amax": (c_int, [c_vp, c_ll, c_vp, c_vp]),
@@ -156,6 +158,7 @@
     "vbg_bn_apply_fold": (c_int, [c_vp, c_vp, c_ll, c_int, c_vp, c_int, c_d, c_vp, c_f, c_f, c_vp, c_vp, c_vp, c_vp, c_vp, c_vp, c_int, c_vp, c_vp, c_vp]),
     "vbg_bn_fold_count": (c_int, [c_vp, c_int, c_int, c_int, c_vp, c_d, c_vp]),
     "vbg_bn_bwd_apply_fold": (c_int, [c_vp, c_vp, c_vp, c_ll, c_int, c_vp, c_vp, c_vp, c_vp, c_int, c_d, c_int, c_vp, c_vp, c_vp, c_vp, c_vp, c_vp]),
+    "vbg_bn_bwd_apply_fold_z": (c_int, [c_vp, c_vp, c_ll, c_int, c_vp, c_vp, c_vp, c_vp, c_vp, c_int, c_d, c_vp, c_vp, c_vp, c_vp, c_vp]),
     "vbg_maxpool3x3s2_fwd": (c_int, [c_vp, c_int, c_int, c_int, c_int, c_vp, c_vp, c_vp]),
     "vbg_maxpool3x3s2_bwd": (c_int, [c_vp, c_vp, c_int, c_int, c_int, c_int, c_int, c_int, c_vp, c_vp]),
     "vbg_avgpool2_fwd": (c_int, [c_vp, c_int, c_int, c_int, c_int, c_vp, c_vp]),
diff --git a/vibertgrid-pytorch_amd/vbg/ops.py b/vibertgrid-pytorch_amd/vbg/ops.py
--- a/vibertgrid-pytorch_amd/vbg/ops.py
+++ b/vibertgrid-pytorch_amd/vbg/ops.py
@@ -82,6 +82,7 @@
 def _untag(t):
     if t is not None:
         t.__dict__.pop("_vbg_amax", None)
+        t.__dict__.pop("_vbg_bn_sums", None)
 
 
 def P(t):
@@ -642,6 +643,15 @@
 
 
 _CONV3_F16 = [os.environ.get("VBG_CONV3_F16", "1") != "0"]
+_BN_FUSE = [os.environ.get("VBG_BN_FUSE", "1") != "0"]
+
+
+def bn_fuse_enabled() -> bool:
+    return _BN_FUSE[0]
+
+
+def set_bn_fuse(on: bool):
+    _BN_FUSE[0] = bool(on)
 _CONV3_MIN_TILES_BWD = [int(os.environ.get("VBG_CONV3_MIN_TILES_BWD", "0"))]
 
 
@@ -698,7 +708,8 @@
     return t
 
 
-def conv3x3(x, w_ohwi, bias=None, out=None, stats=None, accumulate=False, f16x2=False, x_amax=None, nsplit=None, w_planes=None, n_out=None, bn=0):
+def conv3x3(x, w_ohwi, bias=None, out=None, stats=None, accumulate=False, f16x2=False, x_amax=None, nsplit=None, w_planes=None, n_out=None, bn=0,
+            bn_src=None):
     B, H, W, Cs = x.shape
     N = w_ohwi.shape[0] if n_out is None else int(n_out)
     if out is None:
@@ -724,15 +735,24 @@
             _seen("conv3:f16x2")
         if bn == 64:
             _seen("conv3:bn64")
+        if bn_src is not None:
+            _seen("bn:bwd_sums_conv3")
     ev = None
     if _CONV3_PROF[0] is not None:
         ev = (torch.cuda.Event(enable_timing=True), torch.cuda.Event(enable_timing=True))
         ev[0].record()
+    onep = w_planes is not None and _AMP[0] and _AMP_FAST[0]
     if w_planes is not None:
         _seen("conv3:pw")
-        onep = _AMP[0] and _AMP_FAST[0]
         if onep:
             _seen("conv3:onep")
+    if bn_src is not None:
+        assert stats is not None and not accumulate and bias is None
+        z, mean, invstd, gamma, beta = bn_src
+        check(lib.vbg_conv3x3_bn_bwd(P(x), P(w_ohwi) if w_planes is None else None, P(w_planes), P(out), P(stats), bn_slots(), B, H, W, Cs, N,
+                                     2 if onep else int(bool(f16x2)), P(x_amax), P(slab), P(tickets), nz, int(bn), P(z), P(mean), P(invstd),
+                                     P(gamma), P(beta), _stream()), "vbg_conv3x3_bn_bwd")
+    elif w_planes is not None:
         check((lib.vbg_conv3x3_pw_amp if onep else lib.vbg_conv3x3_pw)(P(x), P(w_planes), P(bias), P(out), P(stats), bn_slots() if stats is not None else 0,
                                                                      B, H, W, Cs, N, int(accumulate), P(x_amax), P(slab), P(tickets), nz, int(bn), _stream()),
               "vbg_conv3x3_pw")
@@ -986,7 +1006,7 @@
     return (B * H * W // 128) * ((N + bn - 1) // bn) >= 240
 
 
-def conv2d_dgrad(dy, w_ohwi, x_shape, stride, pad, out=None, accumulate=False, dy_amax=None, w_owner=None):
+def conv2d_dgrad(dy, w_ohwi, x_shape, stride, pad, out=None, accumulate=False, dy_amax=None, w_owner=None, bn_src=None):
     _chk_f32(dy, w_ohwi)
     B, H, W, Cin = x_shape
     Cout, kh, kw, _ = w_ohwi.shape
@@ -997,19 +1017,31 @@
         out = torch.empty(x_shape, device=dy.device, dtype=f32)
     M = B * H * W
     if conv3_ok(B, H, W, Cout, Cin, kh, kw, stride, pad):
+        if bn_src is not None and (accumulate or not bn_fuse_enabled()):
+            bn_src = None
+        sums = bn_zero_slots(dy.device, Cin) if bn_src is not None else None
+        kw_bn = dict(stats=sums, bn_src=bn_src)
         if _CONV3_F16[0]:
             late = conv3_late_choice(B, H, W, Cout, Cin)
+            wp = None
             if late is not None:
                 wp = conv3_planes(w_owner, w_ohwi, True, bn=late[0])
                 if wp is not None:
-                    return conv3x3(dy, w_ohwi, None, out, None, accumulate, f16x2=True, x_amax=dy_amax if dy_amax is not None else amax(dy),
-                                   w_planes=wp, n_out=Cin, nsplit=late[1], bn=late[0])
-            wp = conv3_planes(w_owner, w_ohwi, True) if conv3_pw_ok(B, H, W, Cout, Cin) else None
-            if wp is not None:
-                return conv3x3(dy, w_ohwi, None, out, None, accumulate, f16x2=True, x_amax=dy_amax if dy_amax is not None else amax(dy),
-                               w_planes=wp, n_out=Cin)
-            return conv3x3(dy, conv3x3_wflip(w_ohwi), None, out, None, accumulate, f16x2=True, x_amax=dy_amax if dy_amax is not None else amax(dy))
-        return conv3x3(dy, conv3x3_wflip(w_ohwi), None, out, None, accumulate)
+                    out = conv3x3(dy, w_ohwi, None, out, accumulate=accumulate, f16x2=True, x_amax=dy_amax if dy_amax is not None else amax(dy),
+                                  w_planes=wp, n_out=Cin, nsplit=late[1], bn=late[0], **kw_bn)
+            if wp is None:
+                wp = conv3_planes(w_owner, w_ohwi, True) if conv3_pw_ok(B, H, W, Cout, Cin) else None
+                if wp is not None:
+                    out = conv3x3(dy, w_ohwi, None, out, accumulate=accumulate, f16x2=True, x_amax=dy_amax if dy_amax is not None else amax(dy),
+                                  w_planes=wp, n_out=Cin, **kw_bn)
+                else:
+                    out = conv3x3(dy, conv3x3_wflip(w_ohwi), None, out, accumulate=accumulate, f16x2=True,
+                                  x_amax=dy_amax if dy_amax is not None else amax(dy), **kw_bn)
+        else:
+            out = conv3x3(dy, conv3x3_wflip(w_ohwi), None, out, accumulate=accumulate, **kw_bn)
+        if sums is not None:
+            out._vbg_bn_sums = (sums, bn_src[0].data_ptr(), out._version)
+        return out
     if kh == 1 and kw == 1 and stride == 1 and pad == 0:
         gemm_raw(M, Cin, Cout, dy, Cout, OP_DENSE_K, w_ohwi, Cin, OP_DENSE_R, out, Cin, accumulate=accumulate, splitk=_BWD_SPLIT)
     else:
@@ -1470,10 +1502,28 @@
     return out
 
 
+def bn_bwd_apply_fold_z(dy, z, mean, invstd, gamma, beta, slots, count, dgamma, dbeta, dx_amax=None):
+    M, C_ = z.shape
+    dx = torch.empty_like(z)
+    _seen("bn:bwd_apply_z")
+    check(lib.vbg_bn_bwd_apply_fold_z(P(dy), P(z), M, C_, P(mean), P(invstd), P(gamma), P(beta), P(slots), bn_slots(), float(count), P(dx),
+                                      P(dgamma), P(dbeta), P(dx_amax), _stream()), "vbg_bn_bwd_apply_fold_z")
+    return dx
+
+
+def bn_sums_tag(dy, z):
+    tag = getattr(dy, "_vbg_bn_sums", None)
+    if tag is None:
+        return None
+    sums, z_ptr, version = tag
+    return sums if (z_ptr == z.data_ptr() and dy._version == version) else None
+
+
 def bn_bwd_reduce(dy, y, x, mean, invstd, relu, sums=None):
     M, C_ = x.shape
     if sums is None:
         sums = _bn_workspace(x.device, C_)
+    _seen("bn:bwd_reduce")
     check(lib.vbg_bn_bwd_reduce(P(dy), P(y), P(x), M, C_, P(mean), P(invstd), int(relu), P(sums), _stream()), "vbg_bn_bwd_reduce")
     return sums
 
```
